# lancedb/lance

Measured on AMD Instinct MI355X. Metric: QPS @ recall@10 (SIFT-1M IVF_PQ nlist=256 M=16) + index-build sec, higher is better.
Workload: dtype f32; 1 GPU; SIFT-1M-like 1Mx128 f32, IVF_PQ nlist=256 M=16 nbits=8, build+search on MI355X; n=1000000, d=128, nlist=256, m=16, k=10, nprobes=10, refine_factor=10, parallelism=single

## Files before the change

### lance_amd/csrc/ctx.cpp

```cpp
#include "common.h"

namespace lh {
static thread_local char g_err[1024] = "";
void set_error(const char *fmt, ...) {
  va_list ap;
  va_start(ap, fmt);
  vsnprintf(g_err, sizeof(g_err), fmt, ap);
  va_end(ap);
}
}

void *lance_hip_ctx::scratch(const char *name, size_t bytes) {
  if (bytes == 0) bytes = 16;
  auto it = slots.find(name);
  if (it != slots.end() && it->second.second >= bytes) return it->second.first;
  if (capturing) {
    lh::set_error("scratch '%s' would have to grow to %zu bytes while a search graph is being captured", name, bytes);
    return nullptr;
  }
  if (it != slots.end()) {
    drop_graphs();
    (void)hipStreamSynchronize(stream);
    (void)hipFree(it->second.first);
    slots.erase(it);
// ... 143 lines not shown
}

int lance_hip_malloc(lance_hip_ctx *ctx, size_t bytes, void **out) {
  lh::CtxLock _ctx_lock(ctx);
  LH_REQUIRE(ctx && out, "malloc: NULL argument");
  LH_CHECK_HIP(hipSetDevice(ctx->device));
  hipError_t e = hipMalloc(out, bytes ? bytes : 16);
  if (e != hipSuccess) {
    lh::set_error("hipMalloc(%zu) failed: %s", bytes, hipGetErrorString(e));
    return LANCE_HIP_ENOMEM;
  }
  return LANCE_HIP_OK;
}
int lance_hip_free(lance_hip_ctx *ctx, void *ptr) {
  lh::CtxLock _ctx_lock(ctx);
  LH_REQUIRE(ctx, "ctx is NULL");
  if (ptr) LH_CHECK_HIP(hipFree(ptr));
  return LANCE_HIP_OK;
}
int lance_hip_memcpy_h2d(lance_hip_ctx *ctx, void *dst, const void *src_host, size_t bytes) {
  lh::CtxLock _ctx_lock(ctx);
  LH_REQUIRE(ctx && (bytes == 0 || (dst && src_host)), "memcpy_h2d: NULL argument");
  if (bytes == 0) return LANCE_HIP_OK;
  LH_CHECK_HIP(hipMemcpyAsync(dst, src_host, bytes, hipMemcpyHostToDevice, ctx->stream));
  LH_CHECK_HIP(hipStreamSynchronize(ctx->stream));
  return LANCE_HIP_OK;
}
int lance_hip_memcpy_d2h(lance_hip_ctx *ctx, void *dst_host, const void *src, size_t bytes) {
  lh::CtxLock _ctx_lock(ctx);
  LH_REQUIRE(ctx && (bytes == 0 || (dst_host && src)), "memcpy_d2h: NULL argument");
  if (bytes == 0) return LANCE_HIP_OK;
  LH_CHECK_HIP(hipMemcpyAsync(dst_host, src, bytes, hipMemcpyDeviceToHost, ctx->stream));
  LH_CHECK_HIP(hipStreamSynchronize(ctx->stream));
  return LANCE_HIP_OK;
}

int lance_hip_timing_enable(lance_hip_ctx *ctx, int on) {
  lh::CtxLock _ctx_lock(ctx);
  LH_REQUIRE(ctx, "ctx is NULL");
  ctx->timing = on != 0;
  return LANCE_HIP_OK;
}

int lance_hip_timing_query(lance_hip_ctx *ctx, const char *kernel, double *ms_total, uint64_t *launches) {
  lh::CtxLock _ctx_lock(ctx);
  LH_REQUIRE(ctx && kernel, "timing_query: NULL argument");
  LH_CHECK_HIP(hipStreamSynchronize(ctx->stream));
  if (strncmp(kernel, "count:", 6) == 0) {
    auto it = ctx->stage_counts.find(kernel + 6);
    if (ms_total) *ms_total = 0.0;
    if (launches) *launches = it == ctx->stage_counts.end() ? 0 : it->second;
    return LANCE_HIP_OK;
  }
  auto &t = ctx->timers[kernel];
  for (auto &ev : t.pending) {
    float ms = 0.f;
    if (hipEventElapsedTime(&ms, ev.first, ev.second) == hipSuccess) {
      t.ms += ms;
      t.launches += 1;
    }
    (void)hipEventDestroy(ev.first);
    (void)hipEventDestroy(ev.second);
  }
  t.pending.clear();
  if (ms_total) *ms_total = t.ms;
  if (launches) *launches = t.launches;
  t.ms = 0.0;
  t.launches = 0;
  return LANCE_HIP_OK;
}

}
```

### lance_amd/csrc/group.hip

```cpp
#include "common.h"
#include "kernels.h"

namespace lh {

constexpr int GROUP_ROWS_PER_BLOCK = 1024;

__global__ __launch_bounds__(64) void group_hist_kernel(const uint32_t *__restrict__ ids, int64_t n, int64_t id_stride,
                                                        int k, int nblocks, uint32_t *__restrict__ blockhist,
                                                        const uint8_t *__restrict__ active) {
  extern __shared__ uint32_t hist[];
  const int b = blockIdx.y;
  if (active && !active[b]) return;
  const int blk = blockIdx.x;
  for (int c = threadIdx.x; c < k; c += 64) hist[c] = 0;
  __syncthreads();
  const uint32_t *idb = ids + (int64_t)b * id_stride;
  const int64_t r0 = (int64_t)blk * GROUP_ROWS_PER_BLOCK;
  for (int ch = 0; ch < GROUP_ROWS_PER_BLOCK / 64; ++ch) {
    const int64_t r = r0 + ch * 64 + threadIdx.x;
    if (r < n) {
      const uint32_t key = idb[r];
      if (key < (uint32_t)k) atomicAdd(&hist[key], 1u);
    }
  }
  __syncthreads();
  uint32_t *out = blockhist + (int64_t)b * k * nblocks;
  for (int c = threadIdx.x; c < k; c += 64) out[(int64_t)c * nblocks + blk] = hist[c];
}

__global__ __launch_bounds__(64) void group_scan_blocks_kernel(uint32_t *__restrict__ blockhist, int k, int nblocks,
                                                               uint32_t *__restrict__ totals,
                                                               const uint8_t *__restrict__ active) {
  const int b = blockIdx.y;
  if (active && !active[b]) return;
  const int c = blockIdx.x;
  uint32_t *h = blockhist + ((int64_t)b * k + c) * nblocks;
  const int lane = threadIdx.x;
  uint32_t carry = 0;
  for (int base = 0; base < nblocks; base += 64) {
    const int i = base + lane;
    const uint32_t v = i < nblocks ? h[i] : 0;
    uint32_t incl = v;
#pragma unroll
    for (int off = 1; off < 64; off <<= 1) {
      const uint32_t t = __shfl_up(incl, off, 64);
      if (lane >= off) incl += t;
    }
    if (i < nblocks) h[i] = carry + incl - v;
    carry += __shfl(incl, 63, 64);
  }
  if (lane == 0) totals[(int64_t)b * k + c] = carry;
}
// ... 99 lines not shown
    if (lane == 63) wsum[wave] = incl;
    __syncthreads();
    uint32_t woff = 0;
    for (int w = 0; w < wave; ++w) woff += wsum[w];
    const uint32_t carry = carry_s;
    if (c < k) st[c] = carry + woff + incl - tot;
    __syncthreads();
    if (threadIdx.x == 255) carry_s = carry + woff + incl;
    __syncthreads();
  }
  if (threadIdx.x == 0) st[k] = carry_s;
}

__global__ __launch_bounds__(64) void group_scatter_kernel(const uint32_t *__restrict__ ids, int64_t n, int64_t id_stride,
                                                           int k, int kbits, int nblocks,
                                                           const uint32_t *__restrict__ blockoffs,
                                                           const uint32_t *__restrict__ starts,
                                                           uint32_t *__restrict__ sorted_rows, int64_t out_stride,
                                                           const uint8_t *__restrict__ active) {
  extern __shared__ uint32_t cursor[];
  const int b = blockIdx.y;
  if (active && !active[b]) return;
  const int blk = blockIdx.x;
  const uint32_t *offs = blockoffs + (int64_t)b * k * nblocks;
  const uint32_t *st = starts + (int64_t)b * (k + 1);
  for (int c = threadIdx.x; c < k; c += 64) cursor[c] = st[c] + offs[(int64_t)c * nblocks + blk];
  __syncthreads();
  const uint32_t *idb = ids + (int64_t)b * id_stride;
  uint32_t *outb = sorted_rows + (int64_t)b * out_stride;
  const int lane = threadIdx.x;
  const uint64_t below = lane == 0 ? 0ull : (~0ull >> (64 - lane));
  const int64_t r0 = (int64_t)blk * GROUP_ROWS_PER_BLOCK;
  for (int ch = 0; ch < GROUP_ROWS_PER_BLOCK / 64; ++ch) {
    const int64_t r = r0 + ch * 64 + lane;
    uint32_t key = LANCE_HIP_NONE;
    if (r < n) key = idb[r];
    const bool valid = key < (uint32_t)k;
    uint64_t mask = __ballot(valid);
    for (int bit = 0; bit < kbits; ++bit) {
      const bool one = (key >> bit) & 1u;
      const uint64_t bal = __ballot(one);
      mask &= one ? bal : ~bal;
    }
    uint32_t base = 0;
    if (valid) base = cursor[key];
    __syncthreads();
    if (valid) {
      const uint32_t rank = (uint32_t)__popcll(mask & below);
      outb[base + rank] = (uint32_t)r;
      if (rank == 0) cursor[key] = base + (uint32_t)__popcll(mask);
    }
    __syncthreads();
  }
}

__global__ __launch_bounds__(256) void group_digit_lo_kernel(const uint32_t *__restrict__ ids, int64_t n, int k, uint32_t *__restrict__ out) {
  const int64_t i = (int64_t)blockIdx.x * 256 + threadIdx.x;
  if (i < n) out[i] = ids[i] < (uint32_t)k ? (ids[i] & 255u) : LANCE_HIP_NONE;
}
__global__ __launch_bounds__(256) void group_digit_hi_kernel(const uint32_t *__restrict__ ids, const uint32_t *__restrict__ p1,
                                                             const uint32_t *__restrict__ nvalid, int64_t n, uint32_t *__restrict__ out) {
  const int64_t j = (int64_t)blockIdx.x * 256 + threadIdx.x;
  if (j < n) out[j] = j < (int64_t)*nvalid ? (ids[p1[j]] >> 8) : LANCE_HIP_NONE;
}
__global__ __launch_bounds__(256) void group_compose_kernel(const uint32_t *__restrict__ p1, const uint32_t *__restrict__ p2,
                                                            const uint32_t *__restrict__ nvalid, int64_t n, uint32_t *__restrict__ out) {
  const int64_t j = (int64_t)blockIdx.x * 256 + threadIdx.x;
  if (j < n && j < (int64_t)*nvalid) out[j] = p1[p2[j]];
}
__global__ __launch_bounds__(256) void group_count_kernel(const uint32_t *__restrict__ ids, int64_t n, int k, uint32_t *__restrict__ counts) {
  const int64_t i = (int64_t)blockIdx.x * 256 + threadIdx.x;
  if (i < n && ids[i] < (uint32_t)k) atomicAdd(&counts[ids[i]], 1u);
}

int stable_group(lance_hip_ctx *ctx, const uint32_t *ids, int64_t n, int64_t id_stride, int k, int batches,
                 uint32_t *starts, uint32_t *sorted_rows, int64_t out_stride, const uint8_t *active);

static int stable_group_wide(lance_hip_ctx *ctx, const uint32_t *ids, int64_t n, int k, uint32_t *starts, uint32_t *sorted_rows) {
  LH_REQUIRE(k <= (1 << 22), "stable_group: k=%d not supported (<= 4194304)", k);
  const int k2 = (k + 255) / 256;
  const size_t nn = (size_t)(n > 0 ? n : 1);
  uint32_t *klo = ctx->scratch_t<uint32_t>("group.klo", nn), *khi = ctx->scratch_t<uint32_t>("group.khi", nn);
  uint32_t *p1 = ctx->scratch_t<uint32_t>("group.p1", nn), *p2 = ctx->scratch_t<uint32_t>("group.p2", nn);
  uint32_t *st1 = ctx->scratch_t<uint32_t>("group.st1", 257), *st2 = ctx->scratch_t<uint32_t>("group.st2", (size_t)k2 + 1);
  uint32_t *counts = ctx->scratch_t<uint32_t>("group.counts", (size_t)k);
  if (!klo || !khi || !p1 || !p2 || !st1 || !st2 || !counts) return LANCE_HIP_ENOMEM;
  const unsigned grid = (unsigned)cdiv(nn, 256);
  hipLaunchKernelGGL(group_digit_lo_kernel, dim3(grid), dim3(256), 0, ctx->stream, ids, n, k, klo);
  LH_TRY(stable_group(ctx, klo, n, n, 256, 1, st1, p1, n, nullptr));
  hipLaunchKernelGGL(group_digit_hi_kernel, dim3(grid), dim3(256), 0, ctx->stream, ids, p1, st1 + 256, n, khi);
  LH_TRY(stable_group(ctx, khi, n, n, k2, 1, st2, p2, n, nullptr));
  hipLaunchKernelGGL(group_compose_kernel, dim3(grid), dim3(256), 0, ctx->stream, p1, p2, st1 + 256, n, sorted_rows);
  LH_CHECK_HIP(lh::memset_async(counts, 0, (size_t)k * 4, ctx->stream));
  hipLaunchKernelGGL(group_count_kernel, dim3(grid), dim3(256), 0, ctx->stream, ids, n, k, counts);
  hipLaunchKernelGGL(group_scan_totals_big_kernel, dim3(1), dim3(256), 0, ctx->stream, counts, k, starts);
  LH_CHECK_HIP(hipGetLastError());
  return LANCE_HIP_OK;
}

int stable_group(lance_hip_ctx *ctx, const uint32_t *ids, int64_t n, int64_t id_stride, int k, int batches,
                 uint32_t *starts, uint32_t *sorted_rows, int64_t out_stride, const uint8_t *active) {
  LH_REQUIRE(k > 0, "stable_group: k=%d not supported", k);
  LH_REQUIRE(n < (1ll << 32), "stable_group: n too large");
  if (batches == 0) return LANCE_HIP_OK;
  if (k > 16384) {
    LH_REQUIRE(batches == 1 && active == nullptr, "stable_group: more than 16384 keys only for a single problem");
    return stable_group_wide(ctx, ids, n, k, starts, sorted_rows);
  }
  const int nblocks = (int)cdiv(n > 0 ? n : 1, GROUP_ROWS_PER_BLOCK);
  uint32_t *blockhist = ctx->scratch_t<uint32_t>("group.blockhist", (size_t)batches * k * nblocks);
  uint32_t *totals = ctx->scratch_t<uint32_t>("group.totals", (size_t)batches * k);
  if (!blockhist || !totals) return LANCE_HIP_ENOMEM;
  int kbits = 0;
  while ((1 << kbits) < k) ++kbits;
  const size_t lds = (size_t)k * sizeof(uint32_t);
  hipLaunchKernelGGL(group_hist_kernel, dim3(nblocks, batches), dim3(64), lds, ctx->stream, ids, n, id_stride, k,
                     nblocks, blockhist, active);
  if (k <= 256 && nblocks <= 256) {
    hipLaunchKernelGGL(group_scan_fused_kernel, dim3(batches), dim3(256), 0, ctx->stream, blockhist, k, nblocks, starts, active);
  } else {
    hipLaunchKernelGGL(group_scan_blocks_kernel, dim3(k, batches), dim3(64), 0, ctx->stream, blockhist, k, nblocks, totals, active);
    hipLaunchKernelGGL(group_scan_totals_kernel, dim3(batches), dim3(256), 0, ctx->stream, totals, k, starts, active);
  }
  hipLaunchKernelGGL(group_scatter_kernel, dim3(nblocks, batches), dim3(64), lds, ctx->stream, ids, n, id_stride, k,
                     kbits, nblocks, blockhist, starts, sorted_rows, out_stride, active);
  LH_CHECK_HIP(hipGetLastError());
  return LANCE_HIP_OK;
}

}
```

### lance_amd/csrc/kernels.h

```cpp
#pragma once
#include <stdint.h>

#include "common.h"

namespace lh {

struct PairwiseArgs {
  const void *x_native = nullptr;
  int x_dtype = 0;
  const float *x = nullptr;
  bool lanes32 = false;
  int64_t n = 0;
  int64_t ldx = 0;
  int x_batch_off = 0;
  const float *cent = nullptr;
  int k = 0;
  int64_t cent_batch_stride = 0;
  const float *bias = nullptr;
  int64_t bias_batch_stride = 0;
  uint32_t *ids = nullptr;
  float *dists = nullptr;
  int64_t out_batch_stride = 0;
  uint8_t *codes = nullptr;
  int codes_ld = 0;
// ... 26 lines not shown
int launch_pq_mfma_encode(lance_hip_ctx *ctx, int dtype, const void *x, int64_t n, int d, const float *cent, const uint32_t *part_ids,
                          int residual, const float *codebook, int m, uint8_t *codes);

struct FlatPool {
  const float *x;
  const void *x_native = nullptr;
  int x_dtype = 0;
  const uint64_t *row_ids;
  int64_t r0, r1;
  const float *q;
  int nq, k, cap;
  uint32_t *tkey;
  uint64_t *trid;
  uint32_t *cnt;
  uint32_t *pkeys;
  uint64_t *prids;
  uint32_t *overflow;
  const float *row_sy = nullptr;
  const float *q_norm = nullptr;
};

int launch_wide_filter(lance_hip_ctx *ctx, const FlatPool &fp, int d, int metric);
int build_allow_bits(lance_hip_ctx *ctx, const uint64_t *row_ids, uint64_t n, const uint8_t *allow_by_rowid, uint64_t n_allow, const uint32_t **bits_out);
bool flat_mfma_supported(int metric, int d, int nq, const void *x, const float *q);
int flat_mfma_prepare(lance_hip_ctx *ctx, const float *q, int nq, int d, const uint16_t **qhi, const uint16_t **qlo, const float **qn);
int launch_flat_filter_mfma(lance_hip_ctx *ctx, const FlatPool &e, int d, int metric, const uint16_t *qhi, const uint16_t *qlo, const float *qn);
bool flat_mfma_wide_supported(int metric, int d, int nq, int64_t n, const float *x, const float *q);
int flat_mfma_wide_prepare_rows(lance_hip_ctx *ctx, const float *x, int64_t n, int d, const uint16_t **xb, const float **xn2);
int flat_mfma_wide_prepare_queries(lance_hip_ctx *ctx, const float *q, int nq, int d, const uint16_t **qb, const float **qn2);
int launch_flat_filter_mfma_wide(lance_hip_ctx *ctx, const FlatPool &e, int d, int metric, const uint16_t *xb, const float *xn2, const uint16_t *qb,
                                 const float *qn2);

int launch_assign(lance_hip_ctx *ctx, const PairwiseArgs &p, int d, int metric, int batches);
bool assign_reads_native(PairwiseArgs p, int d, int batches);
bool encode_fused_supported(int dtype, int d, int m, int nbits, const void *x, const float *cent, const float *codebook);
int launch_encode_fused(lance_hip_ctx *ctx, int dtype, const void *x, int64_t n, int d, const float *cent, const uint32_t *part_ids,
                        int residual, const float *codebook, int m, uint8_t *codes);
bool xform_fused_supported(int dtype, int metric, int d, int m, int nbits, int64_t n, int nlist, const void *x, const float *cent,
                           const float *codebook, uint8_t *codes, bool lanes32);
int launch_xform_fused(lance_hip_ctx *ctx, int dtype, int metric, const void *x, int64_t n, int d, const float *cent, int nlist,
                       const float *codebook, int m, uint32_t *part_ids, float *dists, uint8_t *codes, bool round_f16);
bool xform_tail_supported(int d, int m, int nbits, int64_t n, const float *x, const float *cent, const float *codebook);
int launch_xform_tail(lance_hip_ctx *ctx, const float *x, int64_t n, int d, const float *cent, const uint32_t *part_ids, int residual, bool round_f16,
                      const float *codebook, int m, uint8_t *codes);
bool xform_pqtrain_supported(const PairwiseArgs &p, int sd, int batches);
int launch_xform_pqtrain(lance_hip_ctx *ctx, const PairwiseArgs &p, int sd, int batches, uint32_t *fb_cnt, uint32_t *fb_items);
bool xform_assign_supported(const PairwiseArgs &p, int d, int metric, int batches);
int launch_xform_assign(lance_hip_ctx *ctx, const PairwiseArgs &p, int d, int metric);
int launch_xform_sweep_groups(lance_hip_ctx *ctx, int metric, const float *q, uint32_t nq, int d, const float *cent, uint32_t nlist, uint32_t *maxbits,
                              float *gkey, int ng, float *e2, const uint16_t *cpl_ready = nullptr, const uint32_t *maxbits_ready = nullptr);
size_t xform_coarse_planes_elems(uint32_t nlist, int d);
int xform_coarse_planes(lance_hip_ctx *ctx, int metric, const float *cent, uint32_t nlist, int d, uint16_t *cpl, uint32_t *maxbits );
bool coarse_groups_shape(int d, uint32_t nlist);
bool mfma_assign_supported(const PairwiseArgs &p, int d, int batches);
int launch_assign_mfma(lance_hip_ctx *ctx, const PairwiseArgs &p, int d, int metric);
int launch_dist_matrix(lance_hip_ctx *ctx, const PairwiseArgs &p, int d, int metric, int batches);

int stable_group(lance_hip_ctx *ctx, const uint32_t *ids, int64_t n, int64_t id_stride, int k, int batches,
                 uint32_t *starts, uint32_t *sorted_rows, int64_t out_stride, const uint8_t *active);

int kmeans_train_batched(lance_hip_ctx *ctx, int metric, const float *x, int64_t n, int64_t ldx, int x_batch_off, int d,
                         int k, int B, uint32_t max_iters, double tol, float balance_factor_scaled, bool have_init,
                         const uint64_t *seeds, float *cent, double *loss_out, uint32_t *iters_out, bool f16_arith = false);

int kmeans_train_hierarchical(lance_hip_ctx *ctx, int metric, const float *x, int64_t n, int d, int target_k, uint32_t max_iters,
                              double tol, float bf_scaled, int hierarchical_k, uint64_t seed, float *cent_out, uint32_t *n_out,
                              bool f16_arith = false);
int check_dtype(int dtype, const char *what);
int model_dtype(int dtype);
int as_f32(lance_hip_ctx *ctx, int dtype, const void *p, size_t count, const char *slot, const float **out);
int widen_into(lance_hip_ctx *ctx, int dtype, const void *p, size_t count, float *dst);
int from_f32(lance_hip_ctx *ctx, int dtype, const float *src, void *dst, size_t count);
int launch_residual(lance_hip_ctx *ctx, const float *x, int64_t n, int d, const float *cent, const uint32_t *part_ids, float *out, bool f16);


bool pm_supported(const lance_hip_index *ix, uint32_t keff, int has_range, uint32_t nq, uint32_t nprobes);
int ivfpq_scan_merge_pm(lance_hip_ctx *ctx, const lance_hip_index *ix, const float *qs, uint32_t nq, const uint32_t *probes,
                        uint32_t nprobes, uint32_t keff, uint32_t k, bool do_refine, uint64_t *ids, float *dists,
                        uint64_t *cand_rid, uint32_t *cand_cnt, uint32_t *flags, const uint32_t *allow);
int find_partitions_f32(lance_hip_ctx *ctx, int metric, const float *qf, uint32_t nq, uint32_t d, const float *cf, uint32_t nlist,
                        uint32_t nprobes, uint32_t *part_ids, float *dists, bool lanes32);
bool flat_small_supported(int metric, int dtype, uint32_t d, uint32_t nq, uint32_t k, uint64_t n);
int flat_topk_small(lance_hip_ctx *ctx, int metric, int dtype, const void *x, const uint64_t *row_ids, uint64_t n, uint32_t d, const float *q,
                    uint32_t nq, uint32_t k, uint64_t *ids, float *dists, bool *done);
bool coarse_mfma_supported(int metric, int d, uint32_t nq, uint32_t nlist, uint32_t nprobes, bool lanes32, const float *q, const float *cent);
int find_partitions_mfma(lance_hip_ctx *ctx, int metric, const float *q, uint32_t nq, int d, const float *cent, uint32_t nlist, uint32_t nprobes,
                         float *matrix, uint32_t *part_ids, float *dists, const uint16_t *cpl_ready = nullptr, const uint32_t *maxbits_ready = nullptr);
int launch_normalize(lance_hip_ctx *ctx, const float *x, int64_t n, int d, float *out, bool f16);
int launch_normalize_planes(lance_hip_ctx *ctx, const float *x, int64_t n, int d, float *out, bool f16, uint16_t *plane16, int dp, float *n2);

int qscan_index_constants(lance_hip_ctx *ctx, lance_hip_index *ix);
constexpr int QSCAN_SEG_CAP = 256;
struct SelectOut;
bool qscan_supported(const lance_hip_index *ix, uint32_t nq, uint32_t nprobes);
bool qscan_tiled_shape(int m, int sd);
int qscan_classb_to_rescan(lance_hip_ctx *ctx, const uint32_t *tbound, uint32_t nq, uint32_t nprobes, uint32_t *seg_cnt, uint32_t *qovf);
int qscan_nearest_keys(lance_hip_ctx *ctx, const uint32_t *probes, uint32_t nq, uint32_t nprobes, uint32_t *keys, uint32_t nb = 1);
int qscan_item_tables(lance_hip_ctx *ctx, const uint32_t *pair_starts, int nlist, int G, uint32_t *item_start, int4 *desc, uint32_t max_items);
int qscan_group(lance_hip_ctx *ctx, const uint32_t *probes, uint32_t nq, uint32_t nprobes, int nlist, const uint32_t *tglobal,
                uint32_t *keys, uint32_t *tbound, uint32_t *pair_starts, uint32_t *pair_idx, uint32_t *item_start4, int4 *desc4,
                uint32_t max_items4, int G = 4, int dot = 0);
int qbound_launch(lance_hip_ctx *ctx, const lance_hip_index *ix, const float *qs, uint32_t nq, uint32_t keff, const uint32_t *pair_starts0,
                  const uint32_t *pair_idx0, uint32_t *item_start, int4 *desc, uint32_t max_items, uint32_t *tglobal, const uint32_t *allow);
int qscan_launch(lance_hip_ctx *ctx, const lance_hip_index *ix, const float *qs, uint32_t nq, uint32_t nprobes, const uint32_t *pair_idx,
                 const uint32_t *item_start4, const int4 *desc4, uint32_t max_items4, const uint32_t *tbound, uint32_t *seg_cnt,
                 uint32_t *seg_pos, uint32_t *qovf, const uint32_t *allow, const uint32_t *probes = nullptr);
bool qscan_pt_enabled(const lance_hip_index *ix);
int qscan_pt_mode(const lance_hip_index *ix);
int qbound_pt_launch(lance_hip_ctx *ctx, const lance_hip_index *ix, const float *qs, uint32_t nq, uint32_t nprobes, uint32_t keff,
                     const uint32_t *probes, const uint32_t *pair_starts0, const uint32_t *pair_idx0, uint32_t *item_start, int4 *desc,
                     uint32_t max_items, uint32_t *tglobal, const uint32_t *allow);
int qmerge_launch(lance_hip_ctx *ctx, const lance_hip_index *ix, const float *qs, uint32_t nq, const uint32_t *probes, uint32_t nprobes,
// ... 20 lines not shown
```

### lance_amd/csrc/mfma_assign.hip

```cpp
#include <algorithm>
#include <cstdlib>
#include <cstring>

#include <hip/hip_fp16.h>

#include "common.h"
#include "exact.cuh"
#include "kernels.h"
#include "ma_common.cuh"

#pragma clang fp contract(off)

namespace lh {

__global__ __launch_bounds__(64) void ma_prep_kernel(const float *__restrict__ cent, int k, int d, int dp, const float *__restrict__ bias,
                                                     uint16_t *__restrict__ chi, uint16_t *__restrict__ clo, float *__restrict__ cn,
                                                     uint32_t *__restrict__ maxbits ,
                                                     const uint8_t *__restrict__ active) {
  if (active && !active[0]) return;
  const int c = blockIdx.x;
  float s = 0.0f;
  for (int e = threadIdx.x; e < dp; e += 64) {
    const float v = e < d ? cent[(int64_t)c * d + e] : 0.0f;
    const uint32_t hb = bf16_rne_bits(v);
// ... 798 lines not shown
    case 5: ok = ma_launch_ks<5>(ctx, a, metric, dtype, p.lanes32); break;
    case 6: ok = ma_launch_ks<6>(ctx, a, metric, dtype, p.lanes32); break;
    case 7: ok = ma_launch_ks<7>(ctx, a, metric, dtype, p.lanes32); break;
    case 8: ok = ma_launch_ks<8>(ctx, a, metric, dtype, p.lanes32); break;
    default: return LANCE_HIP_EINVAL;
  }
  LH_REQUIRE(ok, "assign: element type %d with metric %d is not on the MFMA path", dtype, metric);
  LH_CHECK_HIP(hipGetLastError());
  return LANCE_HIP_OK;
}

constexpr int CS_CAP = 128;
constexpr int CS_CAP_G = 512;

template <int METRIC>
__device__ __forceinline__ float cs_group_distance(const float *wrow, const float *__restrict__ y, int d, int lane) {
  const int i = lane & 15, full = d / 16 * 16;
  float s = 0.0f, acc = 0.0f;
  if (full != d) {
    float r = 0.0f;
    for (int e = full; e < d; ++e) {
      if constexpr (METRIC == METRIC_DOT) r = r + wrow[e] * y[e];
      else { const float diff = wrow[e] - y[e]; r = r + diff * diff; }
    }
    s = r;
  }
  int ch = 0;
  for (; ch + 128 <= full; ch += 128) {
    float yv[8];
#pragma unroll
    for (int u = 0; u < 8; ++u) yv[u] = y[ch + 16 * u + i];
#pragma unroll
    for (int u = 0; u < 8; ++u) {
      const float xv = wrow[ch + 16 * u + i];
      if constexpr (METRIC == METRIC_DOT) acc = acc + xv * yv[u];
      else { const float diff = xv - yv[u]; acc = acc + diff * diff; }
    }
  }
  for (; ch < full; ch += 16) {
    const float xv = wrow[ch + i], yv = y[ch + i];
    if constexpr (METRIC == METRIC_DOT) acc = acc + xv * yv;
    else { const float diff = xv - yv; acc = acc + diff * diff; }
  }
  float run = 0.0f + acc;
#pragma unroll
  for (int t = 1; t < 16; ++t) {
    const float prev = __builtin_bit_cast(float, __builtin_amdgcn_update_dpp(0, __builtin_bit_cast(int, run), 0x111, 0xF, 0xF, false));
    run = prev + acc;
  }
  const float tot = __shfl(run, (lane & 48) + 15, 64);
  return finish_metric<METRIC>(s + tot);
}

template <int METRIC, bool GROUPS = false>
__global__ __launch_bounds__(256) void coarse_select_kernel(float *__restrict__ sur, const float *__restrict__ e2, const float *__restrict__ q,
                                                            const float *__restrict__ cent, int nq, int nlist, int d, int nprobes,
                                                            uint32_t *__restrict__ part_ids, float *__restrict__ dists,
                                                            uint32_t *__restrict__ n_exact_rows, const float *__restrict__ gkey = nullptr,
                                                            const float *__restrict__ gsec = nullptr, int ng = 0) {
  extern __shared__ __attribute__((aligned(16))) char smem[];
  const int lane = threadIdx.x & 63, wave = threadIdx.x >> 6, grp = lane >> 4;
  const int qi = blockIdx.x * 4 + wave;
  if (qi >= nq) return;
  const int dpad = (d + 3) & ~3;
  constexpr int CAP = GROUPS ? CS_CAP_G : CS_CAP;
  float *wrow = reinterpret_cast<float *>(smem) + (size_t)wave * dpad;
  unsigned long long *ck = reinterpret_cast<unsigned long long *>(smem + (size_t)4 * dpad * 4) + (size_t)wave * CAP;
  uint32_t *cl = reinterpret_cast<uint32_t *>(smem + (size_t)4 * dpad * 4 + (size_t)4 * CAP * 8) + (size_t)wave * CAP;
  const float *qv = q + (int64_t)qi * d;
  for (int e = lane; e < d; e += 64) wrow[e] = qv[e];
  float *row = sur + (int64_t)qi * nlist;
  const float E2 = GROUPS ? e2[qi] * 1.0625f : e2[qi];
  const float *gk = GROUPS ? gkey + (int64_t)qi * 2 * ng : nullptr;
  float m0 = INFINITY, m1 = INFINITY, m2 = INFINITY, m3 = INFINITY;
  bool bad = !(E2 < INFINITY) || !(E2 > 7.888609052210118e-31f);
  auto ins4 = [&](float v) {
    if (v < m3) {
      if (v < m2) {
        m3 = m2;
        if (v < m1) {
          m2 = m1;
          if (v < m0) { m1 = m0; m0 = v; } else m1 = v;
        } else m2 = v;
      } else m3 = v;
    }
  };
  if constexpr (GROUPS) {
    for (int i = lane * 4; i < 2 * ng; i += 256) {
      const f4 v = *reinterpret_cast<const f4 *>(gk + i);
      bad |= (v.x != v.x) | (v.y != v.y);
      ins4(v.x); ins4(v.y);
    }
  } else {
  for (int i = lane; i < nlist; i += 64) {
    const float v = row[i];
    bad |= v != v;
    ins4(v);
  }
  }
  bad = __any(bad);
  float sv4[4] = {m0, m1, m2, m3};
#pragma unroll
  for (int k2 = 2; k2 <= 256; k2 <<= 1) {
#pragma unroll
    for (int dd = k2 >> 1; dd > 0; dd >>= 1) {
      if (dd >= 64) {
        const int jd = dd >> 6;
#pragma unroll
        for (int jr = 0; jr < 4; ++jr) {
          if ((jr & jd) == 0) {
            const bool up = ((jr * 64) & k2) == 0;
            const float lo = fminf(sv4[jr], sv4[jr | jd]), hi = fmaxf(sv4[jr], sv4[jr | jd]);
            sv4[jr] = up ? lo : hi; sv4[jr | jd] = up ? hi : lo;
          }
        }
      } else {
#pragma unroll
        for (int jr = 0; jr < 4; ++jr) {
          const int e = jr * 64 + lane;
          const float o = __shfl_xor(sv4[jr], dd, 64);
          const bool up = (e & k2) == 0, lower = (lane & dd) == 0;
          sv4[jr] = (lower == up) ? fminf(sv4[jr], o) : fmaxf(sv4[jr], o);
        }
      }
    }
  }
// ... 67 lines not shown
    for (int r = 0; r < nprobes; ++r) {
      unsigned long long best = ~0ull;
      for (int i = lane; i < nlist; i += 64) {
        const unsigned long long kk = ((unsigned long long)order_key(row[i]) << 32) | (uint32_t)i;
        if ((!have_last || kk > last) && kk < best) best = kk;
      }
#pragma unroll
      for (int o = 32; o > 0; o >>= 1) { const unsigned long long ob = __shfl_xor(best, o, 64); best = ob < best ? ob : best; }
      if (lane == 0) {
        part_ids[(int64_t)qi * nprobes + r] = (uint32_t)best;
        if (dists) dists[(int64_t)qi * nprobes + r] = key_to_float((uint32_t)(best >> 32));
      }
      last = best; have_last = true;
    }
    return;
  }
  for (uint32_t c0 = 0; c0 < cnt; c0 += 4) {
    const uint32_t ci = c0 + (uint32_t)grp;
    const uint32_t c = ci < cnt ? cl[ci] : cl[0];
    const float v = cs_group_distance<METRIC>(wrow, cent + (int64_t)c * d, d, lane);
    if (ci < cnt && (lane & 15) == 0) ck[ci] = ((unsigned long long)order_key(v) << 32) | c;
  }
  __builtin_amdgcn_wave_barrier();
  unsigned long long v2[2];
  v2[0] = (uint32_t)lane < cnt ? ck[lane] : ~0ull;
  for (uint32_t base = 64;; base += 64) {
    v2[1] = base + (uint32_t)lane < cnt ? ck[base + (uint32_t)lane] : ~0ull;
#pragma unroll
    for (int k2 = 2; k2 <= 128; k2 <<= 1) {
#pragma unroll
      for (int dd = k2 >> 1; dd > 0; dd >>= 1) {
        if (dd >= 64) {
          const unsigned long long a = v2[0], b = v2[1];
          if (a > b) { v2[0] = b; v2[1] = a; }
        } else {
#pragma unroll
          for (int jr = 0; jr < 2; ++jr) {
            const int e = jr * 64 + lane;
            const unsigned long long o = __shfl_xor(v2[jr], dd, 64);
            const bool up = (e & k2) == 0, lower = (lane & dd) == 0;
            v2[jr] = (lower == up) ? (v2[jr] < o ? v2[jr] : o) : (v2[jr] > o ? v2[jr] : o);
          }
        }
      }
    }
    if (base + 64 >= cnt) break;
  }
  if (lane < nprobes) {
    part_ids[(int64_t)qi * nprobes + lane] = (uint32_t)v2[0];
    if (dists) dists[(int64_t)qi * nprobes + lane] = key_to_float((uint32_t)(v2[0] >> 32));
  }
}

bool coarse_mfma_supported(int metric, int d, uint32_t nq, uint32_t nlist, uint32_t nprobes, bool lanes32, const float *q, const float *cent) {
  static const char *env = getenv("LANCE_HIP_MFMA_COARSE");
  static const bool off = env && env[0] == '0', force = env && env[0] == '1';
  if (off || lanes32 || (metric != METRIC_L2 && metric != METRIC_DOT)) return false;
  if (nprobes == 0 || nprobes > 64 || nprobes > nlist) return false;
  if ((reinterpret_cast<uintptr_t>(q) | reinterpret_cast<uintptr_t>(cent)) & 15) return false;
  if (d <= 128) { if (d % 16 != 0 || d < 16 || nlist < 32) return false; }
  else if (d > 4096 || nlist < 64 || d % 4 != 0) return false;
  if (force) return true;
  if (d > 128) return (uint64_t)nq * nlist >= (1ull << 23);
  return (uint64_t)nq * nlist * (uint64_t)d >= (1ull << 27);
}

template <int KS>
static void coarse_launch_narrow(lance_hip_ctx *ctx, const MaArgs &a, int metric, dim3 grid) {
  constexpr int D = KS * 16;
  const size_t lds_x = (size_t)MA_ROWS * (D + 4) * 4;
  const size_t lds_c = (size_t)2 * 2 * MA_CT * (D + 8) * 2 + (size_t)2 * 2 * MA_CT * 4;
  const size_t lds = std::max(lds_x, lds_c);
  if (a.gkey) {
    if (metric == METRIC_DOT) hipLaunchKernelGGL((ma_top3_kernel<KS, METRIC_DOT, float, 2>), grid, dim3(256), lds, ctx->stream, a);
    else hipLaunchKernelGGL((ma_top3_kernel<KS, METRIC_L2, float, 2>), grid, dim3(256), lds, ctx->stream, a);
    return;
  }
  if (metric == METRIC_DOT) hipLaunchKernelGGL((ma_top3_kernel<KS, METRIC_DOT, float, 1>), grid, dim3(256), lds, ctx->stream, a);
  else hipLaunchKernelGGL((ma_top3_kernel<KS, METRIC_L2, float, 1>), grid, dim3(256), lds, ctx->stream, a);
}

static int coarse_groups_from() {
  static const int v = getenv("LANCE_HIP_COARSE_GROUPS") ? atoi(getenv("LANCE_HIP_COARSE_GROUPS")) : 1024;
  return v;
}
bool coarse_groups_shape(int d, uint32_t nlist) {
  static const bool ma = getenv("LANCE_HIP_COARSE_GROUPS_MA") != nullptr;
  return !ma && d <= 128 && d % 16 == 0 && coarse_groups_from() > 0 && nlist >= (uint32_t)std::max(coarse_groups_from(), 256);
}

int find_partitions_mfma(lance_hip_ctx *ctx, int metric, const float *q, uint32_t nq, int d, const float *cent, uint32_t nlist, uint32_t nprobes,
                         float *matrix, uint32_t *part_ids, float *dists, const uint16_t *cpl_ready, const uint32_t *maxbits_ready) {
  const bool wide = d > 128;
  const int dp = wide ? (d + MW_KC - 1) / MW_KC * MW_KC : d;
  const size_t kd = (size_t)nlist * dp;
  uint16_t *chi = ctx->scratch_t<uint16_t>("cq.chi", kd), *clo = ctx->scratch_t<uint16_t>("cq.clo", kd);
  float *cn = ctx->scratch_t<float>("cq.cn", (size_t)nlist);
  uint32_t *maxbits = ctx->scratch_t<uint32_t>("cq.maxbits", 4);
  float *e2 = ctx->scratch_t<float>("cq.e2", (size_t)nq);
  if (!chi || !clo || !cn || !maxbits || !e2) return LANCE_HIP_ENOMEM;
  const int groups_from = coarse_groups_from();
  const bool groups = !wide && groups_from > 0 && nlist >= (uint32_t)std::max(groups_from, 256);
  const int ng = groups ? (int)cdiv(nlist, MA_CT) * 4 : 0;
  float *gkey = nullptr, *gsec = nullptr;
  if (groups) {
    gkey = ctx->scratch_t<float>("cq.gkey", (size_t)nq * 2 * ng);
    gsec = gkey;
    if (!gkey) return LANCE_HIP_ENOMEM;
  }
  LH_CHECK_HIP(lh::memset_async(maxbits, 0, 16, ctx->stream));
  static const bool groups_ma = getenv("LANCE_HIP_COARSE_GROUPS_MA") != nullptr;
  if (groups && !groups_ma) {
    ScopedTimer t(ctx, "dist_matrix");
    LH_TRY(launch_xform_sweep_groups(ctx, metric, q, nq, d, cent, nlist, maxbits, gkey, ng, e2, cpl_ready, maxbits_ready));
  } else {
    ScopedTimer t(ctx, "dist_matrix");
    hipLaunchKernelGGL(ma_prep_kernel, dim3(nlist), dim3(64), 0, ctx->stream, cent, (int)nlist, d, dp, nullptr, chi, clo, cn, maxbits, nullptr);
    MaArgs a;
    a.x = q; a.n = nq; a.ldx = d; a.d = d; a.k = (int)nlist;
    a.chi = chi; a.clo = clo; a.cn = cn; a.bias = nullptr; a.maxbits = maxbits; a.cent = cent;
    a.sur = matrix; a.e2 = e2; a.active = nullptr;
    a.gkey = gkey; a.gsec = gsec; a.ng = ng;
    const unsigned rblocks = (unsigned)cdiv(nq, wide ? MW_ROWS : MA_ROWS);
    const int ntiles = (int)cdiv(nlist, wide ? MW_CT : MA_CT);
    int slices = (int)std::min<uint64_t>((uint64_t)ntiles, std::max<uint64_t>(1, ((uint64_t)2 * ctx->num_cus) / rblocks));
    a.tiles_per_block = (int)cdiv((uint64_t)ntiles, (uint64_t)slices);
    slices = (int)cdiv((uint64_t)ntiles, (uint64_t)a.tiles_per_block);
    const dim3 grid(rblocks, (unsigned)slices);
    if (wide) {
      uint16_t *xhi = ctx->scratch_t<uint16_t>("cq.xhi", (size_t)nq * dp), *xlo = ctx->scratch_t<uint16_t>("cq.xlo", (size_t)nq * dp);
      float *xn2 = ctx->scratch_t<float>("cq.xn2", (size_t)nq);
      if (!xhi || !xlo || !xn2) return LANCE_HIP_ENOMEM;
      a.xhi = xhi; a.xlo = xlo; a.xn2 = xn2; a.dp = dp;
      hipLaunchKernelGGL((ma_split_rows_kernel<float>), dim3((unsigned)cdiv(nq, 4)), dim3(256), 0, ctx->stream, q, (int64_t)nq, (int64_t)d, d, dp, xhi, xlo,
                         xn2, nullptr);
      if (metric == METRIC_DOT) hipLaunchKernelGGL((ma_top3_wide_kernel<METRIC_DOT, true>), grid, dim3(256), 0, ctx->stream, a);
      else hipLaunchKernelGGL((ma_top3_wide_kernel<METRIC_L2, true>), grid, dim3(256), 0, ctx->stream, a);
    } else {
      switch (d / 16) {
        case 1: coarse_launch_narrow<1>(ctx, a, metric, grid); break;
        case 2: coarse_launch_narrow<2>(ctx, a, metric, grid); break;
        case 3: coarse_launch_narrow<3>(ctx, a, metric, grid); break;
        case 4: coarse_launch_narrow<4>(ctx, a, metric, grid); break;
        case 5: coarse_launch_narrow<5>(ctx, a, metric, grid); break;
        case 6: coarse_launch_narrow<6>(ctx, a, metric, grid); break;
        case 7: coarse_launch_narrow<7>(ctx, a, metric, grid); break;
        case 8: coarse_launch_narrow<8>(ctx, a, metric, grid); break;
        default: return LANCE_HIP_EINVAL;
      }
    }
  }
  {
    ScopedTimer t(ctx, "select_probes");
    const int dpad = (d + 3) & ~3;
    const int cap = groups ? CS_CAP_G : CS_CAP;
    const size_t lds = (size_t)4 * dpad * 4 + (size_t)4 * cap * 8 + (size_t)4 * cap * 4;
    if (groups) {
      ctx->count_stage("coarse_groups");
      if (metric == METRIC_DOT)
        hipLaunchKernelGGL((coarse_select_kernel<METRIC_DOT, true>), dim3((unsigned)cdiv(nq, 4)), dim3(256), lds, ctx->stream, matrix, e2, q, cent, (int)nq,
                           (int)nlist, d, (int)nprobes, part_ids, dists, maxbits + 2, gkey, gsec, ng);
      else
        hipLaunchKernelGGL((coarse_select_kernel<METRIC_L2, true>), dim3((unsigned)cdiv(nq, 4)), dim3(256), lds, ctx->stream, matrix, e2, q, cent, (int)nq,
                           (int)nlist, d, (int)nprobes, part_ids, dists, maxbits + 2, gkey, gsec, ng);
    } else if (metric == METRIC_DOT)
      hipLaunchKernelGGL((coarse_select_kernel<METRIC_DOT>), dim3((unsigned)cdiv(nq, 4)), dim3(256), lds, ctx->stream, matrix, e2, q, cent, (int)nq, (int)nlist,
                         d, (int)nprobes, part_ids, dists, maxbits + 2);
    else
      hipLaunchKernelGGL((coarse_select_kernel<METRIC_L2>), dim3((unsigned)cdiv(nq, 4)), dim3(256), lds, ctx->stream, matrix, e2, q, cent, (int)nq, (int)nlist,
                         d, (int)nprobes, part_ids, dists, maxbits + 2);
  }
  static const bool stats = getenv("LANCE_HIP_COARSE_STATS") != nullptr;
  if (stats && !ctx->capturing) {
    uint32_t h[4];
    LH_CHECK_HIP(hipMemcpyAsync(h, maxbits, 16, hipMemcpyDeviceToHost, ctx->stream));
    LH_CHECK_HIP(hipStreamSynchronize(ctx->stream));
    fprintf(stderr, "[coarse] nq=%u nlist=%u nprobes=%u groups=%d: %u queries took the exact path\n", nq, nlist, nprobes, groups ? 1 : 0, h[2]);
  }
  LH_CHECK_HIP(hipGetLastError());
  return LANCE_HIP_OK;
}

}
```

### lance_amd/csrc/search.hip

```cpp
#include <algorithm>
#include <cstdlib>
#include <string>
#include <vector>

#include "common.h"
#include "exact.cuh"
#include "index.h"
#include "kernels.h"
#include "search_common.cuh"

#pragma clang fp contract(off)

namespace lh {

#ifndef LH_SCAN_CAP
#define LH_SCAN_CAP 1024
#endif
#ifndef LH_SCAN_ROUND
#define LH_SCAN_ROUND 512
#endif
#ifndef LH_LUT_BATCH
#define LH_LUT_BATCH 4
#endif
constexpr int SCAN_CAP = LH_SCAN_CAP;
// ... 851 lines not shown
            }
          }
      }
    }
    float oth[8];
#pragma unroll
    for (int e = 0; e < 8; ++e) oth[e] = __shfl_xor(acc[e], 1, 64);
    if (h == 0 && i < P) {
      float tot = 0.0f;
#pragma unroll
      for (int e = 0; e < 8; ++e) tot = tot + acc[e];
#pragma unroll
      for (int e = 0; e < 8; ++e) tot = tot + oth[e];
      tot = 0.0f + tot;
      key[i] = ok ? order_key(finish_metric<METRIC>(tot)) : 0xFFFFFFFFu;
      rid[i] = r; pos[i] = 0;
    }
  }
  __syncthreads();
  refine_write_cand_exact(cand_exact, key, keff, c, qi);
  refine_emit_topk(key, rid, pos, P, c, k, qi, out_ids, out_dists);
}

__global__ __launch_bounds__(256) void raw_to_u8_kernel(const f4 *__restrict__ x, int64_t n16, uint4 *__restrict__ out, uint32_t *__restrict__ bad) {
  bool ok = true;
  for (int64_t i = (int64_t)blockIdx.x * 256 + threadIdx.x; i < n16; i += (int64_t)gridDim.x * 256) {
    uint32_t w[4];
#pragma unroll
    for (int p = 0; p < 4; ++p) {
      const f4 v = x[i * 4 + p];
      uint32_t pk = 0;
#pragma unroll
      for (int e = 0; e < 4; ++e) {
        const uint32_t b = (v[e] >= 0.0f && v[e] < 256.0f) ? (uint32_t)v[e] : 0u;
        ok = ok && (float)b == v[e];
        pk |= b << (8 * e);
      }
      w[p] = pk;
    }
    out[i] = make_uint4(w[0], w[1], w[2], w[3]);
  }
  if (__any(!ok) && (threadIdx.x & 63) == 0) atomicOr(bad, 1u);
}

static bool raw_compact_enabled() {
  static const bool off = getenv("LANCE_HIP_NO_RAW_COMPACT") != nullptr;
  return !off;
}
int coarse_planes_prepare(lance_hip_ctx *ctx, const lance_hip_index *ix_c, int scan_metric) {
  lance_hip_index *ix = const_cast<lance_hip_index *>(ix_c);
  std::lock_guard<std::mutex> lk(ix->lazy_mu);
  if (ix->cq || ctx->capturing) return LANCE_HIP_OK;
  auto *cq = new lance_hip_index::CqConst();
  bool ok = hipMalloc(reinterpret_cast<void **>(&cq->cpl), xform_coarse_planes_elems(ix->nlist, (int)ix->d) * 2) == hipSuccess;
  ok = ok && hipMalloc(reinterpret_cast<void **>(&cq->maxbits), 16) == hipSuccess;
  auto drop = [&]() { if (cq->cpl) (void)hipFree(cq->cpl); if (cq->maxbits) (void)hipFree(cq->maxbits); delete cq; };
  if (!ok) { (void)hipGetLastError(); drop(); return LANCE_HIP_OK; }
  if (lh::memset_async(cq->maxbits, 0, 16, ctx->stream) != hipSuccess ||
      xform_coarse_planes(ctx, scan_metric, ix->centroids, ix->nlist, (int)ix->d, cq->cpl, cq->maxbits) != LANCE_HIP_OK ||
      hipStreamSynchronize(ctx->stream) != hipSuccess) {
    drop();
    set_error("find_partitions: building the centroid planes of the index failed");
    return LANCE_HIP_ERUNTIME;
  }
  ix->cq = cq;
  return LANCE_HIP_OK;
}

const uint8_t *raw_compact_prepare(lance_hip_ctx *ctx, const lance_hip_index *ix_c) {
  lance_hip_index *ix = const_cast<lance_hip_index *>(ix_c);
  if (!raw_compact_enabled() || ix->dtype != LANCE_HIP_F32 || !ix->raw || ix->n_raw == 0 || (ix->d & 15) != 0 ||
      (ix->metric != LANCE_HIP_L2 && ix->metric != LANCE_HIP_DOT) || (reinterpret_cast<uintptr_t>(ix->raw) & 15) != 0)
    return nullptr;
  std::lock_guard<std::mutex> lk(ix->lazy_mu);
  if (ix->raw_compact_state != 0) return ix->raw_compact_state > 0 ? ix->raw_u8 : nullptr;
  if (ctx->capturing) return nullptr;
  const uint64_t bytes = ix->n_raw * (uint64_t)ix->d;
  uint8_t *buf = nullptr;
  uint32_t *bad = ctx->scratch_t<uint32_t>("raw.compact_flag", 1);
  if (!bad || hipMalloc(reinterpret_cast<void **>(&buf), bytes) != hipSuccess) {
    (void)hipGetLastError();
    ix->raw_compact_state = -1;
    return nullptr;
  }
  uint32_t bad_h = 1;
  bool ran = lh::memset_async(bad, 0, 4, ctx->stream) == hipSuccess;
  if (ran) {
    const int64_t n16 = (int64_t)(bytes / 16);
    hipLaunchKernelGGL(raw_to_u8_kernel, dim3((unsigned)std::min<uint64_t>(cdiv((uint64_t)n16, 256), 1u << 20)), dim3(256), 0, ctx->stream,
                       static_cast<const f4 *>(ix->raw), n16, reinterpret_cast<uint4 *>(buf), bad);
    ran = hipGetLastError() == hipSuccess && hipMemcpyAsync(&bad_h, bad, 4, hipMemcpyDeviceToHost, ctx->stream) == hipSuccess &&
          hipStreamSynchronize(ctx->stream) == hipSuccess;
  }
  if (!ran || bad_h != 0) {
    (void)hipFree(buf);
    ix->raw_compact_state = -1;
    return nullptr;
  }
  ix->raw_u8 = buf;
  ix->raw_compact_state = 1;
  return buf;
}


struct ExactArgs {
  ScanArgs s;
  const uint64_t *row_ids;
  int k, refine;
  uint64_t *out_ids;
  float *out_dists;
  uint64_t *cand_rid;
  uint32_t *cand_cnt;
// ... 321 lines not shown
    }
    for (int i = 0; i < 4 && hipGetLastError() != hipSuccess; ++i) {}
  }
  set_error("");
  int prc = plain();
  if (prc == LANCE_HIP_ERUNTIME) {
    (void)hipStreamSynchronize(ctx->stream);
    for (int i = 0; i < 4 && hipGetLastError() != hipSuccess; ++i) {}
    set_error("");
    prc = plain();
  }
  return prc;
}

static int ivfpq_search_enqueue_impl(lance_hip_ctx *ctx, const lance_hip_index *ix, const float *q, uint32_t nq, uint32_t k,
                                     uint32_t nprobes, uint32_t refine_factor, int has_range, float lower, float upper,
                                     uint64_t *ids, float *dists, uint32_t **flags_out, const uint32_t *allow) {
  LH_REQUIRE(k > 0, "search: k must be > 0");
  if (nprobes > ix->nlist) nprobes = ix->nlist;
  LH_REQUIRE(ix->nlist <= 8192 || nprobes <= 2048, "search: nprobes=%u > 2048 with more than 8192 partitions is not supported", nprobes);
  LH_REQUIRE(nprobes > 0, "search: nprobes must be > 0");
  const uint32_t rf = refine_factor == 0 ? 1 : refine_factor;
  const uint64_t keff64 = (uint64_t)k * rf;
  LH_REQUIRE(keff64 <= 8192, "search: k * refine_factor = %llu > 8192 is not supported", (unsigned long long)keff64);
  const uint32_t keff = (uint32_t)keff64;
  const bool fast = keff <= (uint32_t)SCAN_MAX_KEFF;
  const bool do_refine = refine_factor >= 1;
  LH_REQUIRE(!do_refine || ix->raw != nullptr, "search: refine_factor needs raw vectors (lance_hip_index_set_raw)");
  const int d = (int)ix->d, m = (int)ix->m, sd = d / m, nlist = (int)ix->nlist;
  const int scan_metric = ix->metric == LANCE_HIP_COSINE ? LANCE_HIP_L2 : ix->metric;

  uint32_t *flags = ctx->scratch_t<uint32_t>("search.flags", (size_t)nq + 1);
  if (!flags) return LANCE_HIP_ENOMEM;
  LH_CHECK_HIP(lh::memset_async(flags, 0, ((size_t)nq + 1) * 4, ctx->stream));
  uint32_t *n_fallback = flags + nq;
  ctx->last_replay_counter = n_fallback;
  if (flags_out) *flags_out = flags;
  if (nq == 0) return LANCE_HIP_OK;

  const float *qs = q;
  if (ix->metric == LANCE_HIP_COSINE) {
    float *qn = ctx->scratch_t<float>("search.qnorm", (size_t)nq * d);
    if (!qn) return LANCE_HIP_ENOMEM;
    LH_TRY(launch_normalize(ctx, q, (int64_t)nq, d, qn, ix->dtype == LANCE_HIP_F16));
    qs = qn;
  }
  float *matrix = ctx->scratch_t<float>("search.matrix", (size_t)nq * nlist);
  uint32_t *probes = ctx->scratch_t<uint32_t>("search.probes", (size_t)nq * nprobes);
  if (!matrix || !probes) return LANCE_HIP_ENOMEM;
  const bool coarse_l32 = ix->dtype == LANCE_HIP_F16 && scan_metric == LANCE_HIP_DOT && d > 16;
  if (coarse_mfma_supported(scan_metric, d, nq, (uint32_t)nlist, nprobes, coarse_l32, qs, ix->centroids)) {
    const uint16_t *cpl = nullptr;
    const uint32_t *cmb = nullptr;
    if (coarse_groups_shape(d, (uint32_t)nlist)) {
      LH_TRY(coarse_planes_prepare(ctx, ix, scan_metric));
      if (ix->cq) { cpl = ix->cq->cpl; cmb = ix->cq->maxbits; }
    }
    LH_TRY(find_partitions_mfma(ctx, scan_metric, qs, nq, d, ix->centroids, (uint32_t)nlist, nprobes, matrix, probes, nullptr, cpl, cmb));
  } else {
    PairwiseArgs pa;
    pa.x = qs; pa.n = nq; pa.ldx = d; pa.cent = ix->centroids; pa.k = nlist; pa.matrix = matrix;
    pa.lanes32 = coarse_l32;
    LH_TRY(launch_dist_matrix(ctx, pa, d, scan_metric, 1));
    ScopedTimer t(ctx, "select_probes");
    launch_select_probes(ctx, matrix, nlist, (int)nprobes, (int)nq, probes, nullptr);
  }
  uint64_t *cand_rid = nullptr;
  uint32_t *cand_cnt = nullptr;
  if (do_refine) {
    cand_rid = ctx->scratch_t<uint64_t>("search.cand_rid", (size_t)nq * keff);
    cand_cnt = ctx->scratch_t<uint32_t>("search.cand_cnt", nq);
    if (!cand_rid || !cand_cnt) return LANCE_HIP_ENOMEM;
  }
  static const bool no_pm = getenv("LANCE_HIP_NO_PM") != nullptr;
  const uint64_t pm_min_pairs = qscan_tiled_shape(m, sd) ? 2048 : 4096;
  const bool use_pm = fast && !no_pm && pm_supported(ix, keff, has_range, nq, nprobes) && (uint64_t)nq * nprobes >= pm_min_pairs;
  int nsplit = 1;
  if (nq < (uint32_t)(2 * ctx->num_cus)) {
    nsplit = (int)std::min<uint64_t>({8ull, (uint64_t)nprobes, cdiv(2ull * ctx->num_cus, nq)});
    if (nsplit < 1) nsplit = 1;
  }
  const size_t nblk = (size_t)nq * nsplit;
  uint32_t *ckeys = nullptr, *cpos = nullptr, *ccnt = nullptr;
  if (!use_pm) {
    ckeys = ctx->scratch_t<uint32_t>("search.ckeys", nblk * SCAN_LCAP);
    cpos = ctx->scratch_t<uint32_t>("search.cpos", nblk * SCAN_LCAP);
    ccnt = ctx->scratch_t<uint32_t>("search.ccnt", nblk);
    if (!ckeys || !cpos || !ccnt) return LANCE_HIP_ENOMEM;
  }
  ScanArgs a;
  {
    a.q = qs; a.probes = probes; a.centroids = ix->centroids; a.codebook = ix->codebook;
    a.part_offsets = ix->part_offsets; a.codes = ix->codes;
    a.d = d; a.m = m; a.sd = sd; a.nprobes = (int)nprobes; a.nsplit = nsplit; a.keff = (int)keff;
    a.nbits = (int)ix->nbits;
    a.residual = scan_metric == LANCE_HIP_L2 ? 1 : 0;
    a.round_f16 = ix->dtype == LANCE_HIP_F16 ? 1 : 0;
    a.lanes32 = (ix->dtype == LANCE_HIP_F16 && scan_metric == LANCE_HIP_DOT && sd > 16) ? 1 : 0;
    a.has_range = has_range;
    a.allow = allow;
    a.lo_key = 0; a.hi_key = 0xFFFFFFFFu;
    if (has_range) {
      uint32_t lb, ub;
      memcpy(&lb, &lower, 4); memcpy(&ub, &upper, 4);
      a.lo_key = (lb & 0x80000000u) ? ~lb : (lb | 0x80000000u);
      a.hi_key = (ub & 0x80000000u) ? ~ub : (ub | 0x80000000u);
    }
// ... 53 lines not shown

int find_partitions_f32(lance_hip_ctx *ctx, int metric, const float *qf, uint32_t nq, uint32_t d, const float *cf, uint32_t nlist,
                        uint32_t nprobes, uint32_t *part_ids, float *dists, bool lanes32) {
  if (nprobes > nlist) nprobes = nlist;
  LH_REQUIRE(nlist <= 8192 || nprobes <= 2048, "find_partitions: nprobes=%u > 2048 with more than 8192 partitions is not supported", nprobes);
  if (nq == 0 || nprobes == 0) return LANCE_HIP_OK;
  float *matrix = ctx->scratch_t<float>("search.matrix", (size_t)nq * nlist);
  if (!matrix) return LANCE_HIP_ENOMEM;
  const int km = metric == LANCE_HIP_COSINE ? LANCE_HIP_L2 : metric;
  if (coarse_mfma_supported(km, (int)d, nq, nlist, nprobes, lanes32, qf, cf)) {
    LH_TRY(find_partitions_mfma(ctx, km, qf, nq, (int)d, cf, nlist, nprobes, matrix, part_ids, dists));
  } else {
    PairwiseArgs pa;
    pa.x = qf; pa.n = nq; pa.ldx = d;
    pa.cent = cf; pa.k = (int)nlist; pa.matrix = matrix;
    pa.lanes32 = lanes32;
    LH_TRY(launch_dist_matrix(ctx, pa, (int)d, km, 1));
    launch_select_probes(ctx, matrix, (int)nlist, (int)nprobes, (int)nq, part_ids, dists);
  }
  LH_CHECK_HIP(hipGetLastError());
  LH_CHECK_HIP(hipStreamSynchronize(ctx->stream));
  return LANCE_HIP_OK;
}

static int check_flags(lance_hip_ctx *ctx, const uint32_t *flags, uint32_t nq) {
  std::vector<uint32_t> fh(nq);
  LH_CHECK_HIP(hipMemcpyAsync(fh.data(), flags, (size_t)nq * 4, hipMemcpyDeviceToHost, ctx->stream));
  LH_CHECK_HIP(hipStreamSynchronize(ctx->stream));
  uint32_t n_over = 0, n_amb = 0, n_bad = 0;
  for (uint32_t i = 0; i < nq; ++i) { n_over += (fh[i] & FLAG_OVERFLOW) ? 1 : 0; n_amb += (fh[i] & FLAG_AMBIGUOUS) ? 1 : 0; n_bad += (fh[i] & FLAG_BADROW) ? 1 : 0; }
  if (n_bad) {
    set_error("search: refine met row ids beyond the %s raw vectors given to lance_hip_index_set_raw (%u queries): the raw array must be "
              "indexed by the stored row ids", "attached", n_bad);
    return LANCE_HIP_EINVAL;
  }
  if (n_over || n_amb) {
    set_error("search: internal error, %u overflow / %u ambiguous queries were not resolved by the exact kernel", n_over, n_amb);
    return LANCE_HIP_ERUNTIME;
  }
  return LANCE_HIP_OK;
}

}

using namespace lh;

extern "C" {

int lance_hip_index_prewarm(lance_hip_ctx *ctx, lance_hip_index *idx) {
  lh::CtxLock _ctx_lock(ctx);
  LH_REQUIRE(ctx && idx, "index_prewarm: NULL argument");
  LH_CHECK_HIP(hipSetDevice(ctx->device));
  if (idx->m > 0 && idx->nbits == 8) LH_TRY(mscan_prewarm(ctx, idx));
  if (coarse_groups_shape((int)idx->d, idx->nlist) && (reinterpret_cast<uintptr_t>(idx->centroids) & 15) == 0)
    LH_TRY(coarse_planes_prepare(ctx, idx, idx->metric == LANCE_HIP_COSINE ? LANCE_HIP_L2 : idx->metric));
  (void)raw_compact_prepare(ctx, idx);
  LH_CHECK_HIP(hipStreamSynchronize(ctx->stream));
  return LANCE_HIP_OK;
}

int lance_hip_find_partitions(lance_hip_ctx *ctx, int dtype, int metric, const void *q, uint32_t nq, uint32_t d,
                              const void *centroids, uint32_t nlist, uint32_t nprobes, uint32_t *part_ids, float *dists) {
  lh::CtxLock _ctx_lock(ctx);
  LH_REQUIRE(ctx && q && centroids && part_ids, "find_partitions: NULL argument");
  LH_TRY(check_dtype(dtype, "find_partitions"));
  LH_REQUIRE(nlist > 0 && nlist <= 65536, "find_partitions: nlist=%u not supported in this version (1..65536)", nlist);
  LH_CHECK_HIP(hipSetDevice(ctx->device));
  const float *qf, *cf;
  LH_TRY(as_f32(ctx, dtype, q, (size_t)nq * d, "f16.q", &qf));
  LH_TRY(as_f32(ctx, model_dtype(dtype), centroids, (size_t)nlist * d, "f16.cent", &cf));
  return find_partitions_f32(ctx, metric, qf, nq, d, cf, nlist, nprobes, part_ids, dists, dtype == LANCE_HIP_F16 && metric == LANCE_HIP_DOT && d > 16);
}

int lance_hip_ivfpq_search_async(lance_hip_ctx *ctx, const lance_hip_index *idx, const void *q, uint32_t nq, uint32_t k,
                                 uint32_t nprobes, uint32_t refine_factor, uint64_t *ids, float *dists) {
  lh::CtxLock _ctx_lock(ctx);
  LH_REQUIRE(ctx && idx && (nq == 0 || (q && ids && dists)), "search: NULL argument");
  LH_REQUIRE(ctx->device == idx->device, "search: context and index live on different devices");
  LH_CHECK_HIP(hipSetDevice(ctx->device));
  const float *qf;
  LH_TRY(as_f32(ctx, idx->dtype, q, (size_t)nq * idx->d, "f16.q", &qf));
  return ivfpq_search_enqueue(ctx, idx, qf, nq, k, nprobes, refine_factor, 0, 0.f, 0.f, ids, dists, nullptr, nullptr);
}

int lance_hip_ivfpq_search(lance_hip_ctx *ctx, const lance_hip_index *idx, const void *q, uint32_t nq, uint32_t k,
                           uint32_t nprobes, uint32_t refine_factor, uint64_t *ids, float *dists) {
  lh::CtxLock _ctx_lock(ctx);
  LH_REQUIRE(ctx && idx && (nq == 0 || (q && ids && dists)), "search: NULL argument");
  LH_REQUIRE(ctx->device == idx->device, "search: context and index live on different devices");
  LH_CHECK_HIP(hipSetDevice(ctx->device));
  uint32_t *flags = nullptr;
  const float *qf;
  LH_TRY(as_f32(ctx, idx->dtype, q, (size_t)nq * idx->d, "f16.q", &qf));
  LH_TRY(ivfpq_search_enqueue(ctx, idx, qf, nq, k, nprobes, refine_factor, 0, 0.f, 0.f, ids, dists, &flags, nullptr));
  return check_flags(ctx, flags, nq);
}

int lance_hip_ivfpq_search_candidates(lance_hip_ctx *ctx, const lance_hip_index *idx, const void *q, uint32_t nq, uint32_t keff, uint32_t nprobes,
                                      uint64_t *ids, float *pq_dists, float *exact_dists) {
  lh::CtxLock _ctx_lock(ctx);
  LH_REQUIRE(ctx && idx && (nq == 0 || (q && ids && pq_dists)), "search_candidates: NULL argument");
  LH_REQUIRE(ctx->device == idx->device, "search_candidates: context and index live on different devices");
  LH_REQUIRE(idx->m != 0, "search_candidates: not an IVF_PQ index");
  LH_REQUIRE(!exact_dists || idx->raw != nullptr, "search_candidates: exact distances need raw vectors (lance_hip_index_set_raw)");
  LH_CHECK_HIP(hipSetDevice(ctx->device));
  if (nq == 0) return LANCE_HIP_OK;
  uint32_t *flags = nullptr;
// ... 136 lines not shown
```

### lance_amd/csrc/search_common.cuh

```cuda
#pragma once
#include <hip/hip_runtime.h>
#include <stdint.h>

#include "exact.cuh"

namespace lh {

constexpr uint32_t FLAG_OVERFLOW = 1u, FLAG_AMBIGUOUS = 2u, FLAG_BADROW = 4u;
constexpr int SCAN_LCAP = 256;
constexpr int SCAN_MAX_KEFF = 128;

__device__ __forceinline__ bool row_allowed(const uint32_t *__restrict__ allow, uint32_t pos) {
  return allow == nullptr || ((allow[pos >> 5] >> (pos & 31u)) & 1u) != 0u;
}

static inline int next_pow2(int v) { int p = 1; while (p < v) p <<= 1; return p; }

__device__ __forceinline__ uint32_t find_partition_dev(const uint32_t *__restrict__ offs, int nlist, uint32_t slot) {
  int lo = 0, hi = nlist;
  while (hi - lo > 1) {
    const int mid = (lo + hi) >> 1;
    if (offs[mid] <= slot) lo = mid; else hi = mid;
  }
  return (uint32_t)lo;
}

template <int BS = 256>
__device__ __forceinline__ void bitonic_sort_kr(uint32_t *key, uint64_t *rid, uint32_t *pos, int P) {
  for (int k2 = 2; k2 <= P; k2 <<= 1) {
    for (int j = k2 >> 1; j > 0; j >>= 1) {
      for (int i = threadIdx.x; i < P / 2; i += BS) {
        const int ix = 2 * j * (i / j) + (i % j);
        const int px = ix + j;
        const bool up = (ix & k2) == 0;
        const uint32_t kx = key[ix], ky = key[px];
        const uint64_t rx = rid[ix], ry = rid[px];
        const bool gt = kx > ky || (kx == ky && rx > ry);
        if (gt == up) {
          key[ix] = ky; key[px] = kx; rid[ix] = ry; rid[px] = rx;
          const uint32_t t = pos[ix]; pos[ix] = pos[px]; pos[px] = t;
        }
      }
      __syncthreads();
    }
  }
}

struct SelectOut {
  int keff, k, refine;
  uint64_t *out_ids;
  float *out_dists;
  uint64_t *cand_rid;
  uint32_t *cand_cnt;
  uint32_t *flags;
  const uint32_t *part_offsets;
  int nlist;
};

template <int BS = 256>
__device__ __forceinline__ void select_and_emit(const SelectOut &o, int q, uint32_t *key, uint64_t *rid, uint32_t *pos, int total,
                                                int *s_amb) {
  const int got = min(total, o.keff);
  if (total > o.keff && key[o.keff] == key[o.keff - 1]) {
    const uint32_t tf = key[o.keff - 1];
    int lo = o.keff, hi = total;
    while (lo < hi) { const int mid = (lo + hi) >> 1; if (key[mid] <= tf) lo = mid + 1; else hi = mid; }
    const int L = lo;
    for (int i = threadIdx.x; i < L; i += BS) {
      const uint32_t pi = find_partition_dev(o.part_offsets, o.nlist, pos[i]);
      const uint32_t a = o.part_offsets[pi], b = o.part_offsets[pi + 1];
      int same = 0;
      for (int j = 0; j < L; ++j) same += (pos[j] >= a && pos[j] < b) ? 1 : 0;
      if (same > o.keff) *s_amb = 1;
    }
    __syncthreads();
    if (threadIdx.x == 0 && *s_amb) atomicOr(&o.flags[q], FLAG_AMBIGUOUS);
  }
// ... 46 lines not shown
```

### lance_amd/csrc/search_ms.hip

```cpp
#include <algorithm>
#include <cmath>
#include <cstdio>
#include <cstdlib>
#include <cstring>
#include <vector>

#include "common.h"
#include "exact.cuh"
#include "index.h"
#include "kernels.h"
#include "search_common.cuh"
#include "q_common.cuh"

namespace lh {

typedef _Float16 ms_h8 __attribute__((ext_vector_type(8)));
typedef _Float16 ms_h4 __attribute__((ext_vector_type(4)));
typedef float ms_f16v __attribute__((ext_vector_type(16)));

constexpr float MS_SE = 30000.0f;
constexpr float MS_SLACK_CAP = 1500.0f;
constexpr int MS_CUT_SHIFT = 6;
typedef __attribute__((address_space(1))) const void *ms_gptr;
typedef __attribute__((address_space(3))) void *ms_lptr;
// ... 212 lines not shown
    uint32_t v = 0;
    if (i < nlist) {
      const uint32_t qp = pair_starts[i + 1] - pair_starts[i], np = part_offsets[i + 1] - part_offsets[i];
      const MsSplit sp = ms_split(qp, np, rs_rows, rs2_rows);
      v = sp.npb * sp.nrs;
      for (uint32_t pb = 0; pb < sp.npb; pb += max(1u, sp.npb - 1u)) {
        const uint32_t pairs = min(sp.blk, qp - pb * sp.blk), npb_same = (pb + 1 == sp.npb) ? 1u : sp.npb - 1u;
        if (sp.nrs > 0) atomicAdd(&hist[ms_work_class(ms_row_count(0u, np, rs_rows, rs2_rows), pairs, cls_rows)], npb_same);
        if (sp.nrs > 2) atomicAdd(&hist[ms_work_class(rs2_rows, pairs, cls_rows)], npb_same * (sp.nrs - 2u));
        if (sp.nrs > 1) atomicAdd(&hist[ms_work_class(ms_row_count(sp.nrs - 1u, np, rs_rows, rs2_rows), pairs, cls_rows)], npb_same);
        if (sp.npb == 1) break;
      }
    }
    uint32_t incl = v;
#pragma unroll
    for (int off = 1; off < 64; off <<= 1) {
      const uint32_t t = __shfl_up(incl, off, 64);
      if (lane >= off) incl += t;
    }
    if (lane == 63) wsum[wave] = incl;
    __syncthreads();
    uint32_t woff = 0;
    for (int w = 0; w < wave; ++w) woff += wsum[w];
    const uint32_t carry = carry_s;
    if (i < nlist) slice_start[i] = carry + woff + incl - v;
    __syncthreads();
    if (threadIdx.x == 255) carry_s = carry + woff + incl;
    __syncthreads();
  }
  if (threadIdx.x == 0) {
    slice_start[nlist] = carry_s;
    uint32_t run = 0;
    for (int c = 0; c < 32; ++c) { cls_cursor[c] = run; run += hist[c]; }
  }
}

__global__ __launch_bounds__(256) void ms_slice_desc_kernel(const uint32_t *__restrict__ slice_start, const uint32_t *__restrict__ pair_starts,
                                                            const uint32_t *__restrict__ part_offsets, int nlist, uint32_t rs_rows, uint32_t rs2_rows, uint32_t cls_rows,
                                                            MsSlice *__restrict__ slices, uint32_t *__restrict__ cls_cursor, uint32_t *__restrict__ order) {
  const int part = blockIdx.x * 4 + (threadIdx.x >> 6), lane = threadIdx.x & 63;
  if (part >= nlist) return;
  const uint32_t s0 = slice_start[part], s1 = slice_start[part + 1];
  if (s1 == s0) return;
  const uint32_t off = part_offsets[part], np = part_offsets[part + 1] - off;
  const uint32_t gs = pair_starts[part], qp = pair_starts[part + 1] - gs;
  const MsSplit sp = ms_split(qp, np, rs_rows, rs2_rows);
  for (uint32_t t = (uint32_t)lane; t < s1 - s0; t += 64u) {
    const uint32_t pb = t / sp.nrs, rs = t - pb * sp.nrs;
    MsSlice u;
    u.off = off; u.np = np; u.row_begin = ms_row_begin(rs, rs_rows, rs2_rows); u.row_count = ms_row_count(rs, np, rs_rows, rs2_rows);
    u.gs = gs + pb * sp.blk; u.qp = min(sp.blk, qp - pb * sp.blk); u.pad0 = u.pad1 = 0u;
    slices[s0 + t] = u;
    order[atomicAdd(&cls_cursor[ms_work_class(u.row_count, u.qp, cls_rows)], 1u)] = s0 + t;
  }
}

struct MscanArgs {
  const uint32_t *order;
  const MsSlice *slices;
  const uint32_t *slice_start;
  uint32_t *slice_ctr;
  const uint8_t *codes;
  const _Float16 *cbh;
  const float *row_cn2;
  const _Float16 *rh;
  const f4 *prm;
  const f2 *prm2;
  uint32_t nan_slot;
  int nlist, nprobes;
  uint32_t *seg_cnt, *seg_pos;
  uint2 *seg_pv = nullptr;
  uint32_t *ovf;
  const uint32_t *allow;
#ifdef LH_TIMING_EXPERIMENTS
  int dbg = 0;
#endif
  unsigned long long *prof_slices = nullptr;
  unsigned long long *prof = nullptr;
};

#ifdef LH_TIMING_EXPERIMENTS
#define MS_DBG(p) ((p).dbg)
#else
#define MS_DBG(p) 0
#endif

constexpr int MS_QH = 64;
template <int SD, int KS, bool PROF = false>
__global__ __launch_bounds__(1024, 4) void ivfpq_mscan_kernel(MscanArgs p) {
  constexpr int D = KS * 16;
  constexpr int M = D / SD;
  constexpr int RB = D * 2;
  constexpr int CPR = RB / 16;
  constexpr int RPK = 256 / RB;
  constexpr int SPI = 16384 / RB;
  __shared__ __attribute__((aligned(16))) char sB[MS3_PB * RB];
  __shared__ __attribute__((aligned(16))) float sLim[MS3_PB];
  __shared__ __attribute__((aligned(16))) uint32_t sPair[MS3_PB];
  __shared__ __attribute__((aligned(8))) uint2 sQ[16][2][MS_QH + 1];
  __shared__ uint32_t s_slice, s_chunk;
  const int lane = threadIdx.x & 63, wave = __builtin_amdgcn_readfirstlane((int)(threadIdx.x >> 6));
  const int j = lane & 31, g = lane >> 5;
  const uint32_t nslices = p.slice_start[p.nlist];

  uint2 *const qw = &sQ[wave][0][0];
  uint32_t cur = 0;
// ... 541 lines not shown
    mc->sum_rs += rs; mc->max_rs = std::max(mc->max_rs, rs);
  }
  if (hipGetLastError() != hipSuccess || hipStreamSynchronize(ctx->stream) != hipSuccess) {
    drop();
    set_error("matrix-core scan: building the index constants failed");
    return LANCE_HIP_ERUNTIME;
  }
  if (dot) {
    float rm; memcpy(&rm, &rowmax_bits, 4);
    mc->cmax = (float)(std::sqrt((double)rm) / (double)mc->sigma * 1.0001);
    if (!(mc->cmax > 0.0f) || !std::isfinite(mc->cmax)) mc->cmax = mc->cmax_full;
  }
  mc->usable = true;
  ix->ms = mc;
  return LANCE_HIP_OK;
}

int mscan_launch(lance_hip_ctx *ctx, const lance_hip_index *ix_c, const float *qs, uint32_t nq, uint32_t nprobes, const uint32_t *probes,
                 const uint32_t *pair_starts, const uint32_t *pair_idx, const uint32_t *tbound, uint32_t *seg_cnt, uint32_t *seg_pos,
                 uint32_t *qovf, const uint32_t *allow, uint32_t **qslack_out, float **seg_val_out, float **seg_scale_out) {
  lance_hip_index *ix = const_cast<lance_hip_index *>(ix_c);
  int sd = 0, ks = 0;
  if (!ms_shape(ix, &sd, &ks)) return LH_NOT_TAKEN;
  LH_TRY(mscan_prepare(ctx, ix));
  if (!ix->ms->usable) return LH_NOT_TAKEN;
  const int d = (int)ix->d, nlist = (int)ix->nlist;
  const size_t npairs = (size_t)nq * nprobes;
  const uint64_t cap = (uint64_t)ix->ms->sum_rs + (uint64_t)ix->ms->max_rs * cdiv(npairs, MS3_PB) + 8;
  _Float16 *rh = reinterpret_cast<_Float16 *>(ctx->scratch("ms.rh", (npairs + 32) * (size_t)d * 2));
  f4 *prm = reinterpret_cast<f4 *>(ctx->scratch("ms.prm", (npairs + 32) * 16));
  f2 *prm2 = reinterpret_cast<f2 *>(ctx->scratch("ms.prm2", npairs * 8));
  uint32_t *qslack = ctx->scratch_t<uint32_t>("ms.qslack", nq);
  uint32_t *slice_start = ctx->scratch_t<uint32_t>("ms.slice_start", (size_t)nlist + 2 + 32);
  MsSlice *slices = reinterpret_cast<MsSlice *>(ctx->scratch("ms.slices", cap * sizeof(MsSlice)));
  uint32_t *order = ctx->scratch_t<uint32_t>("ms.order", cap);
  float *seg_val = ctx->scratch_t<float>("ms.seg_val", npairs * Q_CAP * 2);
  uint32_t *ovf = ctx->scratch_t<uint32_t>("q.ovf", npairs + 1);
  if (!rh || !prm || !prm2 || !qslack || !slice_start || !slices || !order || !seg_val || !ovf) return LANCE_HIP_ENOMEM;
  uint32_t *slice_ctr = slice_start + nlist + 1, *cls_cursor = slice_ctr + 1;
  const uint32_t nan_slot = (uint32_t)npairs + 1u;
  {
    ScopedTimer t(ctx, "q_residual");
    LH_CHECK_HIP(lh::memset_multi(ctx->stream, {{seg_cnt, 0, npairs * 4}, {qovf, 0, (size_t)nq * 4}, {qslack, 0, (size_t)nq * 4}, {ovf, 0, 4}}));
    MsPrepArgs pa;
    pa.q = qs; pa.centroids = ix->centroids; pa.pair_idx = pair_idx; pa.pair_starts = pair_starts; pa.probes = probes; pa.tbound = tbound;
    pa.d = d; pa.nprobes = (int)nprobes; pa.nlist = nlist; pa.round_f16 = ix->dtype == LANCE_HIP_F16 ? 1 : 0;
    pa.sigma = ix->ms->sigma; pa.rh = rh; pa.prm = prm; pa.qslack = qslack; pa.seg_cnt = seg_cnt; pa.qovf = qovf; pa.ovf = ovf;
    pa.nan_slot = nan_slot; pa.prm2 = prm2;
    pa.dot = ix->metric == LANCE_HIP_DOT ? 1 : 0; pa.cmax = ix->ms->cmax; pa.cmax_full = ix->ms->cmax_full; pa.cmaxp = ix->ms->cmaxp; pa.mu = ix->cb_mean; pa.m = (int)ix->m;
    hipLaunchKernelGGL(ms_prep_kernel, dim3((unsigned)cdiv(npairs, 4 * MS_PPW)), dim3(256), 0, ctx->stream, pa);
    const uint32_t rs_rows = (uint32_t)ms_rows_per_slice(), rs2_rows = (uint32_t)ms_rows_per_slice2();
    static const bool no_order = getenv("LANCE_HIP_MS_NOORDER") != nullptr;
    const uint32_t cls_rows = no_order ? 0x40000000u : rs_rows;
    hipLaunchKernelGGL(ms_slice_table_kernel, dim3(1), dim3(256), 0, ctx->stream, pair_starts, ix->part_offsets, nlist, rs_rows, rs2_rows, cls_rows, slice_start,
                       slice_ctr, cls_cursor);
    hipLaunchKernelGGL(ms_slice_desc_kernel, dim3((unsigned)cdiv((uint64_t)nlist, 4)), dim3(256), 0, ctx->stream, slice_start, pair_starts, ix->part_offsets,
                       nlist, rs_rows, rs2_rows, cls_rows, slices, cls_cursor, order);
  }
  ScopedTimer t(ctx, "ivfpq_scan_c1");
  ScopedTimer tm(ctx, "ivfpq_mscan");
  MscanArgs a;
  a.order = order; a.slices = slices; a.slice_start = slice_start; a.slice_ctr = slice_ctr; a.codes = ix->codes;
  a.cbh = reinterpret_cast<const _Float16 *>(ix->ms->cbh); a.row_cn2 = ix->ms->row_cn2; a.rh = rh; a.prm = prm; a.prm2 = prm2;
  a.nan_slot = nan_slot; a.nlist = nlist; a.nprobes = (int)nprobes;
  a.seg_cnt = seg_cnt; a.seg_pos = seg_pos; a.seg_pv = reinterpret_cast<uint2 *>(seg_val); a.ovf = ovf; a.allow = allow;
#ifdef LH_TIMING_EXPERIMENTS
  static const int dbg = [] {
    const int v = getenv("LANCE_HIP_MS_DBG") ? atoi(getenv("LANCE_HIP_MS_DBG")) : 0;
    if (v) fprintf(stderr, "lance_hip: LANCE_HIP_MS_DBG=%d -- timing experiment, search RESULTS ARE WRONG\n", v);
    return v;
  }();
  a.dbg = dbg;
#endif
  static const int grid_env = getenv("LANCE_HIP_MS_GRID") ? atoi(getenv("LANCE_HIP_MS_GRID")) : 0;
  const unsigned grid = (unsigned)std::min<uint64_t>((uint64_t)(grid_env > 0 ? std::min(grid_env, ctx->num_cus) : ctx->num_cus), cap);
  static const bool prof = getenv("LANCE_HIP_MS_PROF") != nullptr;
  if (prof && sd == 8 && ks == 8 && !ctx->capturing) {
    a.prof = ctx->scratch_t<unsigned long long>("ms.prof", 8);
    if (!a.prof) return LANCE_HIP_ENOMEM;
    LH_CHECK_HIP(lh::memset_async(a.prof, 0, 64, ctx->stream));
    a.prof_slices = ctx->scratch_t<unsigned long long>("ms.prof_slices", cap);
    if (!a.prof_slices) return LANCE_HIP_ENOMEM;
    LH_CHECK_HIP(lh::memset_async(a.prof_slices, 0, cap * 8, ctx->stream));
    hipLaunchKernelGGL((ivfpq_mscan_kernel<8, 8, true>), dim3(grid), dim3(1024), 0, ctx->stream, a);
    unsigned long long h[8];
    LH_CHECK_HIP(hipMemcpyAsync(h, a.prof, 64, hipMemcpyDeviceToHost, ctx->stream));
    LH_CHECK_HIP(hipStreamSynchronize(ctx->stream));
    {
      std::vector<unsigned long long> st(cap);
      std::vector<MsSlice> sl(cap);
      std::vector<uint32_t> ord(cap), ss((size_t)nlist + 1);
      (void)hipMemcpy(st.data(), a.prof_slices, cap * 8, hipMemcpyDeviceToHost);
      (void)hipMemcpy(sl.data(), slices, cap * sizeof(MsSlice), hipMemcpyDeviceToHost);
      (void)hipMemcpy(ord.data(), order, cap * 4, hipMemcpyDeviceToHost);
      (void)hipMemcpy(ss.data(), slice_start, ((size_t)nlist + 1) * 4, hipMemcpyDeviceToHost);
      const uint32_t ns = ss[nlist];
      std::vector<uint32_t> idx(ns);
      for (uint32_t i = 0; i < ns; ++i) idx[i] = i;
      std::sort(idx.begin(), idx.end(), [&](uint32_t x, uint32_t y) { return st[x] > st[y]; });
      double tot = 0, totw = 0;
      for (uint32_t i = 0; i < ns; ++i) { tot += (double)st[i]; totw += (double)sl[ord[i]].row_count * sl[ord[i]].qp; }
      fprintf(stderr, "[ms prof] %u slices, mean %.0f ticks, mean ticks per 1000 cells %.2f; slowest (taken#, ticks, rows, pairs, ticks per 1000 cells):", ns, tot / ns, tot / totw * 1e3);
      for (uint32_t t = 0; t < std::min<uint32_t>(ns, 12); ++t) {
        const uint32_t i = idx[t];
        fprintf(stderr, " (%u, %llu, %u, %u, %.2f)", i, st[i], sl[ord[i]].row_count, sl[ord[i]].qp, (double)st[i] / ((double)sl[ord[i]].row_count * sl[ord[i]].qp) * 1e3);
      }
      fprintf(stderr, " | last taken:");
      for (uint32_t i = ns > 12 ? ns - 12 : 0; i < ns; ++i)
        fprintf(stderr, " (%u, %llu, %u, %u)", i, st[i], sl[ord[i]].row_count, sl[ord[i]].qp);
      fprintf(stderr, "\n");
// ... 55 lines not shown
```

### lance_amd/csrc/search_pm.hip

```cpp
#include <algorithm>
#include <cstdio>
#include <cstdlib>
#include <cstdlib>
#include <vector>

#include "common.h"
#include "exact.cuh"
#include "index.h"
#include "kernels.h"
#include "search_common.cuh"
#include "pm_common.cuh"

#pragma clang fp contract(off)

namespace lh {

#ifndef LH_PM_BS
#define LH_PM_BS 512
#endif
#ifndef LH_PM_STATIC_LUT
#define LH_PM_STATIC_LUT 0
#endif
constexpr int PM_BS = LH_PM_BS;
constexpr int PM_CAP = PM_BS + 256;
// ... 30 lines not shown
__global__ __launch_bounds__(256) void pm_keys_kernel(const uint32_t *__restrict__ probes, int64_t npairs, int nprobes, int nlist,
                                                      uint32_t *__restrict__ keys) {
  const int64_t i = (int64_t)blockIdx.x * 256 + threadIdx.x;
  if (i >= npairs) return;
  keys[i] = probes[i] + ((i % nprobes) == 0 ? 0u : (uint32_t)nlist);
}

__global__ __launch_bounds__(256) void pm_item_table_kernel(const uint32_t *__restrict__ pair_starts, int nlist,
                                                            uint32_t *__restrict__ item_start) {
  __shared__ uint32_t wsum[4];
  __shared__ uint32_t carry_s;
  const int lane = threadIdx.x & 63, wave = threadIdx.x >> 6;
  if (threadIdx.x == 0) carry_s = 0;
  __syncthreads();
  for (int base = 0; base < nlist; base += 256) {
    const int i = base + threadIdx.x;
    const uint32_t v = i < nlist ? (pair_starts[i + 1] - pair_starts[i] + 1) / 2 : 0;
    uint32_t incl = v;
#pragma unroll
    for (int off = 1; off < 64; off <<= 1) {
      const uint32_t t = __shfl_up(incl, off, 64);
      if (lane >= off) incl += t;
    }
    if (lane == 63) wsum[wave] = incl;
    __syncthreads();
    uint32_t woff = 0;
    for (int w = 0; w < wave; ++w) woff += wsum[w];
    const uint32_t carry = carry_s;
    if (i < nlist) item_start[i] = carry + woff + incl - v;
    __syncthreads();
    if (threadIdx.x == 255) carry_s = carry + woff + incl;
    __syncthreads();
  }
  if (threadIdx.x == 0) item_start[nlist] = carry_s;
}

__global__ __launch_bounds__(256) void pm_item_desc_kernel(const uint32_t *__restrict__ item_start, const uint32_t *__restrict__ pair_starts,
                                                           const uint32_t *__restrict__ pair_idx, int nvp, int nlist, int nprobes, uint32_t max_items,
                                                           int4 *__restrict__ desc) {
  const uint32_t item = blockIdx.x * 256 + threadIdx.x;
  if (item >= max_items) return;
  int4 dsc = make_int4(-1, -1, -1, 0);
  if (item < item_start[nvp]) {
    int vp = (int)find_partition_dev(item_start, nvp, item);
    while (item_start[vp + 1] <= item) ++vp;
    const uint32_t g = item - item_start[vp];
    const uint32_t ps = pair_starts[vp], pe = pair_starts[vp + 1];
    const uint32_t i0 = ps + 2 * g;
    dsc.x = vp % nlist;
    dsc.y = (int)(pair_idx[i0] / (uint32_t)nprobes);
    dsc.z = i0 + 1 < pe ? (int)(pair_idx[i0 + 1] / (uint32_t)nprobes) : -1;
  }
  desc[item] = dsc;
}

template <int SD, int METRIC, int MU, int RPL, int CAP>
__device__ __forceinline__ void pm_scan_item(const PmArgs &p, const uint32_t item) {
  extern __shared__ __attribute__((aligned(16))) char smem[];
  constexpr int m = MU * 16;
  constexpr int Q = SD / 4;
  const int dpad = (p.d + 3) & ~3;
  float *r0 = reinterpret_cast<float *>(smem);
  float *r1 = r0 + dpad;
#if LH_PM_STATIC_LUT
  __shared__ __attribute__((aligned(16))) f2 lut2[m * 256];
  uint32_t *ck0 = reinterpret_cast<uint32_t *>(r1 + dpad);
#else
  f2 *lut2 = reinterpret_cast<f2 *>(r1 + dpad);
  uint32_t *ck0 = reinterpret_cast<uint32_t *>(lut2 + m * 256);
#endif
  uint32_t *cp0 = ck0 + CAP;
  uint32_t *ck1 = cp0 + CAP;
  uint32_t *cp1 = ck1 + CAP;
  uint32_t *sorted = cp1 + CAP;
  uint32_t *misc = sorted + PM_BS;
  __shared__ int s_part, s_q0, s_q1, s_valid;

  const int cb_c = threadIdx.x & 255, cb_half = threadIdx.x >> 8;
  constexpr int MH = m / (PM_BS / 256), MA = MH / 2;
  f4 cbA[MA][Q];
#pragma unroll
  for (int i = 0; i < MA; ++i) {
    const f4 *src = reinterpret_cast<const f4 *>(p.codebook + ((int64_t)(cb_half * MH + i) * 256 + cb_c) * SD);
#pragma unroll
    for (int u = 0; u < Q; ++u) cbA[i][u] = src[u];
  }

  if (threadIdx.x == 0) {
    const uint32_t it = p.loop ? item : item + (p.cls == 1 ? p.item_start[p.nlist] : 0u);
    const int valid = p.loop ? 1 : (it < p.item_start[(p.cls == 0 ? 1 : 2) * p.nlist]);
    int4 dsc = make_int4(0, -1, -1, 0);
    if (valid) dsc = p.desc[it];
    const int part = dsc.x, q0 = dsc.y, q1 = dsc.z;
    s_valid = valid; s_part = part; s_q0 = q0; s_q1 = q1;
    misc[0] = 0; misc[2] = 0; misc[5] = 0;
  }
  const long long pt0 = p.prof ? clock64() : 0;
  __syncthreads();
  if (!s_valid) return;
  const long long pt1 = p.prof ? clock64() : 0;
  const int part = s_part, q0 = s_q0, q1 = s_q1;
  const bool has1 = q1 >= 0;
  float qa_v = 0.0f, qb_v = 0.0f, cen_v = 0.0f;
  if ((int)threadIdx.x < p.d) {
    qa_v = p.q[(int64_t)q0 * p.d + threadIdx.x];
    qb_v = p.q[(int64_t)(has1 ? q1 : q0) * p.d + threadIdx.x];
// ... 365 lines not shown
static int ivfpq_scan_merge_q(lance_hip_ctx *ctx, const lance_hip_index *ix, const float *qs, uint32_t nq, const uint32_t *probes,
                              uint32_t nprobes, uint32_t keff, uint32_t k, bool do_refine, uint64_t *ids, float *dists,
                              uint64_t *cand_rid, uint32_t *cand_cnt, uint32_t *flags, const uint32_t *allow) {
  const int d = (int)ix->d, m = (int)ix->m, sd = d / m, nlist = (int)ix->nlist;
  const size_t npairs = (size_t)nq * nprobes;
  const uint32_t max_items2 = (uint32_t)(npairs / 2 + 2 * nlist + 2);
  const uint32_t max_items4 = (uint32_t)(npairs / 4 + nlist + 2);
  uint32_t *keys = ctx->scratch_t<uint32_t>("pm.keys", npairs);
  uint32_t *pair_starts = ctx->scratch_t<uint32_t>("pm.pair_starts", (size_t)2 * nlist + 1);
  uint32_t *pair_idx = ctx->scratch_t<uint32_t>("pm.pair_idx", npairs);
  uint32_t *item_start = ctx->scratch_t<uint32_t>("pm.item_start", (size_t)2 * nlist + 1);
  int4 *desc = ctx->scratch_t<int4>("pm.desc", max_items2);
  uint32_t *pair_starts0 = ctx->scratch_t<uint32_t>("q.pair_starts0", (size_t)nlist + 1);
  static const uint32_t dot_nb_env = getenv("LANCE_HIP_DOT_BOUND_LISTS") ? (uint32_t)std::max(1, atoi(getenv("LANCE_HIP_DOT_BOUND_LISTS"))) : 3u;
  static const uint32_t l2_nb_env = getenv("LANCE_HIP_BOUND_LISTS") ? (uint32_t)std::max(1, atoi(getenv("LANCE_HIP_BOUND_LISTS"))) : 1u;
  static const bool no_msbound_env = getenv("LANCE_HIP_NO_MSBOUND") != nullptr || getenv("LANCE_HIP_EXACT_BOUND") != nullptr;
  const uint32_t l2_nb = (!no_msbound_env && l2_nb_env > 1 && mscan_supported(ix, nq, nprobes) && qscan_pt_mode(ix) != 2) ? l2_nb_env : 1u;
  const uint32_t nb0 = std::min<uint32_t>(std::min<uint32_t>(ix->metric == LANCE_HIP_DOT ? dot_nb_env : l2_nb, 4u), nprobes);
  const uint32_t max_items0 = (uint32_t)((size_t)nq * nb0 / 2 + nlist + 2);
  uint32_t *pair_idx0 = ctx->scratch_t<uint32_t>("q.pair_idx0", (size_t)nq * nb0);
  uint32_t *item_start0 = ctx->scratch_t<uint32_t>("q.item_start0", (size_t)nlist + 1);
  int4 *desc0 = ctx->scratch_t<int4>("q.desc0", max_items0);
  uint32_t *item_start4 = ctx->scratch_t<uint32_t>("q.item_start4", (size_t)nlist + 1);
  int4 *desc4 = ctx->scratch_t<int4>("q.desc4", max_items4);
  uint32_t *tglobal = ctx->scratch_t<uint32_t>("pm.tglobal", (size_t)nq * 4);
  uint32_t *seg_cnt = ctx->scratch_t<uint32_t>("q.seg_cnt", npairs);
  uint32_t *seg_pos = ctx->scratch_t<uint32_t>("q.seg_pos", npairs * QSCAN_SEG_CAP);
  uint64_t pool_max = qscan_tiled_shape(m, sd) ? 65536 : 8192;
  while (pool_max > 8192 && (uint64_t)nq * pool_max * 8 > (1ull << 30)) pool_max /= 2;
  int pool_cap = (int)std::min<uint64_t>(pool_max, std::max<uint64_t>(512, (uint64_t)nprobes * (keff + 28)));
  pool_cap = (pool_cap + 255) & ~255;
  uint32_t *pool_key = ctx->scratch_t<uint32_t>("pm.pool_key", (size_t)nq * pool_cap);
  uint32_t *pool_pos = ctx->scratch_t<uint32_t>("pm.pool_pos", (size_t)nq * pool_cap);
  if (!keys || !pair_starts || !pair_idx || !item_start || !desc || !pair_starts0 || !pair_idx0 || !item_start0 || !desc0 || !item_start4 ||
      !desc4 || !tglobal || !seg_cnt || !seg_pos || !pool_key || !pool_pos)
    return LANCE_HIP_ENOMEM;
  uint32_t *pool_cnt = tglobal + nq, *tbound = tglobal + 2 * (size_t)nq, *qovf = tglobal + 3 * (size_t)nq;
  LH_CHECK_HIP(lh::memset_multi(ctx->stream, {{tglobal, 0xFF, (size_t)nq * 4}, {pool_cnt, 0, (size_t)nq * 4}}));
  PmArgs a;
  a.q = qs; a.probes = probes;
  a.centroids = ix->centroids; a.codebook = ix->codebook; a.part_offsets = ix->part_offsets; a.codes = ix->codes;
  a.d = d; a.m = m; a.nprobes = (int)nprobes; a.nlist = nlist; a.keff = (int)keff;
  const bool dot = ix->metric == LANCE_HIP_DOT;
  a.residual = dot ? 0 : 1;
  a.round_f16 = ix->dtype == LANCE_HIP_F16 ? 1 : 0;
  a.prof = nullptr;
  a.tglobal = tglobal; a.pool_key = pool_key; a.pool_pos = pool_pos; a.pool_cnt = pool_cnt; a.pool_cap = pool_cap; a.flags = flags;
  a.unbounded = 0; a.loop = 0; a.allow = allow;
  const bool tiled = qscan_tiled_shape(m, sd);
  static const bool exact_bound_env = getenv("LANCE_HIP_EXACT_BOUND") != nullptr;
  const bool exact_bound = exact_bound_env && !tiled && !dot;
  {
    ScopedTimer t(ctx, "pm_group");
    LH_TRY(qscan_nearest_keys(ctx, probes, nq, nprobes, keys, nb0));
    LH_TRY(stable_group(ctx, keys, (int64_t)nq * nb0, (int64_t)nq * nb0, nlist, 1, pair_starts0, pair_idx0, (int64_t)nq * nb0, nullptr));
    if (exact_bound) {
      hipLaunchKernelGGL(pm_item_table_kernel, dim3(1), dim3(256), 0, ctx->stream, pair_starts0, nlist, item_start0);
      hipLaunchKernelGGL(pm_item_desc_kernel, dim3((unsigned)cdiv(max_items0, 256)), dim3(256), 0, ctx->stream, item_start0, pair_starts0, pair_idx0,
                         nlist, nlist, 1, max_items0, desc0);
    }
  }
  if (exact_bound) {
    ScopedTimer t(ctx, "ivfpq_scan_c0");
    a.pair_starts = pair_starts0; a.pair_idx = pair_idx0; a.item_start = item_start0; a.desc = desc0;
    a.cls = 0; a.bound_pass = 1;
    const size_t lds = pm_lds_base(d, m) + (size_t)PM_CAP_BOUND * 16;
    const bool ok = launch_pm_sd<METRIC_L2>(ctx, a, sd, (unsigned)(nq / 2 + nlist + 1), lds);
    LH_REQUIRE(ok, "partition-major scan: unsupported shape (m=%d, sd=%d)", m, sd);
  } else if (!dot && qscan_pt_mode(ix) == 2) {
    ScopedTimer t(ctx, "ivfpq_scan_c0");
    LH_TRY(qbound_pt_launch(ctx, ix, qs, nq, nprobes, keff, probes, pair_starts0, pair_idx0, item_start0, desc0, (uint32_t)(nq / 4 + nlist + 2), tglobal,
                            allow));
  } else {
    ScopedTimer t(ctx, "ivfpq_scan_c0");
    int mb_rc = LH_NOT_TAKEN;
    if (mscan_supported(ix, nq, nprobes))
      mb_rc = msbound_launch(ctx, ix, qs, nq, keff, pair_starts0, pair_idx0, item_start0, desc0, (uint32_t)((size_t)nq * nb0 / 4 + nlist + 2), tglobal, allow, nb0);
    if (mb_rc < 0) return mb_rc;
    if (mb_rc == LH_NOT_TAKEN && dot) return LH_NOT_TAKEN;
    if (mb_rc == LH_NOT_TAKEN) LH_TRY(qbound_launch(ctx, ix, qs, nq, keff, pair_starts0, pair_idx0, item_start0, desc0, (uint32_t)(nq / 4 + nlist + 2), tglobal, allow));
  }
  {
    ScopedTimer t(ctx, "pm_group");
    LH_TRY(qscan_group(ctx, probes, nq, nprobes, nlist, tglobal, keys, tbound, pair_starts, pair_idx, item_start4, desc4, max_items4, 4, dot ? 1 : 0));
    hipLaunchKernelGGL(pm_item_table_kernel, dim3(1), dim3(256), 0, ctx->stream, pair_starts, 2 * nlist, item_start);
    hipLaunchKernelGGL(pm_item_desc_kernel, dim3((unsigned)cdiv(max_items2, 256)), dim3(256), 0, ctx->stream, item_start, pair_starts, pair_idx,
                       2 * nlist, nlist, (int)nprobes, max_items2, desc);
  }
  uint32_t *qslack = nullptr;
  float *seg_val = nullptr, *seg_scale = nullptr;
  int ms_rc = LH_NOT_TAKEN;
  if (mscan_supported(ix, nq, nprobes))
    ms_rc = mscan_launch(ctx, ix, qs, nq, nprobes, probes, pair_starts, pair_idx, tbound, seg_cnt, seg_pos, qovf, allow, &qslack, &seg_val, &seg_scale);
  if (ms_rc < 0) return ms_rc;
  if (ms_rc == LH_NOT_TAKEN && dot) return LH_NOT_TAKEN;
  if (ms_rc == LH_NOT_TAKEN) {
    qslack = nullptr; seg_val = nullptr; seg_scale = nullptr;
    LH_TRY(qscan_launch(ctx, ix, qs, nq, nprobes, pair_idx, item_start4, desc4, max_items4, tbound, seg_cnt, seg_pos, qovf, allow, probes));
  }
  static const bool q_stats = getenv("LANCE_HIP_Q_STATS") != nullptr;
  if (q_stats) {
    std::vector<uint32_t> sc(npairs), tb(nq);
    (void)hipMemcpyAsync(sc.data(), seg_cnt, npairs * 4, hipMemcpyDeviceToHost, ctx->stream);
    (void)hipMemcpyAsync(tb.data(), tbound, (size_t)nq * 4, hipMemcpyDeviceToHost, ctx->stream);
    (void)hipStreamSynchronize(ctx->stream);
    uint64_t tot = 0, ovf = 0, mx = 0, nb = 0, r0 = 0;
    for (size_t i = 0; i < npairs; ++i) { tot += std::min<uint32_t>(sc[i], QSCAN_SEG_CAP); ovf += sc[i] > (uint32_t)QSCAN_SEG_CAP; mx = std::max<uint64_t>(mx, sc[i]); if (i % nprobes == 0) r0 += sc[i]; }
    for (uint32_t i = 0; i < nq; ++i) nb += tb[i] == 0xFFFFFFFFu;
    fprintf(stderr, "[qscan] nq=%u nprobes=%u keff=%u survivors/query %.1f (nearest partition %.1f) max segment %llu overflowed segments %llu class-B queries %llu\n",
            nq, nprobes, keff, (double)tot / nq, (double)r0 / nq, (unsigned long long)mx, (unsigned long long)ovf, (unsigned long long)nb);
  }
  if (tiled) {
    ScopedTimer t(ctx, "ivfpq_scan_cb");
    LH_TRY(qscan_classb_to_rescan(ctx, tbound, nq, nprobes, seg_cnt, qovf));
  } else {
    ScopedTimer t(ctx, "ivfpq_scan_cb");
    a.pair_starts = pair_starts; a.pair_idx = pair_idx; a.item_start = item_start; a.desc = desc;
    a.cls = 1; a.bound_pass = 0; a.unbounded = 1; a.loop = 1;
    const size_t lds = pm_lds_base(d, m) + (size_t)PM_CAP * 16;
    const unsigned grid = (unsigned)std::min<uint64_t>((uint64_t)ctx->num_cus * 3, (uint64_t)max_items2);
    const bool ok = dot ? launch_pm_sd<METRIC_DOT>(ctx, a, sd, grid, lds) : launch_pm_sd<METRIC_L2>(ctx, a, sd, grid, lds);
    LH_REQUIRE(ok, "partition-major scan: unsupported shape (m=%d, sd=%d)", m, sd);
  }
  {
    SelectOut o;
    o.keff = (int)keff; o.k = (int)k; o.refine = do_refine ? 1 : 0;
    o.out_ids = ids; o.out_dists = dists; o.cand_rid = cand_rid; o.cand_cnt = cand_cnt; o.flags = flags;
    o.part_offsets = ix->part_offsets; o.nlist = nlist;
    ScopedTimer t(ctx, "ivfpq_merge");
    LH_TRY(qmerge_launch(ctx, ix, qs, nq, probes, nprobes, tbound, tglobal, seg_cnt, seg_pos, qovf, pool_key, pool_pos, pool_cnt, pool_cap, o, allow, qslack, seg_val, seg_scale));
  }
  LH_CHECK_HIP(hipGetLastError());
  return LANCE_HIP_OK;
}

int ivfpq_scan_merge_pm(lance_hip_ctx *ctx, const lance_hip_index *ix, const float *qs, uint32_t nq, const uint32_t *probes,
                        uint32_t nprobes, uint32_t keff, uint32_t k, bool do_refine, uint64_t *ids, float *dists,
                        uint64_t *cand_rid, uint32_t *cand_cnt, uint32_t *flags, const uint32_t *allow) {
  const int d = (int)ix->d, m = (int)ix->m, sd = d / m, nlist = (int)ix->nlist;
  const int scan_metric = ix->metric == LANCE_HIP_COSINE ? LANCE_HIP_L2 : ix->metric;
  if (!pm_nobound() && qscan_supported(ix, nq, nprobes)) {
    const int rc = ivfpq_scan_merge_q(ctx, ix, qs, nq, probes, nprobes, keff, k, do_refine, ids, dists, cand_rid, cand_cnt, flags, allow);
    if (rc != LH_NOT_TAKEN) return rc;
  }
  const size_t npairs = (size_t)nq * nprobes;
  uint32_t *pair_starts = ctx->scratch_t<uint32_t>("pm.pair_starts", (size_t)2 * nlist + 1);
  uint32_t *pair_idx = ctx->scratch_t<uint32_t>("pm.pair_idx", npairs);
  uint32_t *item_start = ctx->scratch_t<uint32_t>("pm.item_start", (size_t)2 * nlist + 1);
  uint32_t *tglobal = ctx->scratch_t<uint32_t>("pm.tglobal", (size_t)nq * 2);
  int pool_cap = (int)std::min<uint64_t>(8192, std::max<uint64_t>(512, (uint64_t)nprobes * (keff + 28)));
  pool_cap = (pool_cap + 255) & ~255;
  uint32_t *pool_key = ctx->scratch_t<uint32_t>("pm.pool_key", (size_t)nq * pool_cap);
  uint32_t *pool_pos = ctx->scratch_t<uint32_t>("pm.pool_pos", (size_t)nq * pool_cap);
  if (!pair_starts || !pair_idx || !item_start || !tglobal || !pool_key || !pool_pos) return LANCE_HIP_ENOMEM;
  uint32_t *pool_cnt = tglobal + nq;
  LH_CHECK_HIP(lh::memset_multi(ctx->stream, {{tglobal, 0xFF, (size_t)nq * 4}, {pool_cnt, 0, (size_t)nq * 4}}));
  uint32_t *keys = ctx->scratch_t<uint32_t>("pm.keys", npairs);
  const uint32_t max_items = (uint32_t)(npairs / 2 + 2 * nlist + 2);
  int4 *desc = ctx->scratch_t<int4>("pm.desc", max_items);
  if (!keys || !desc) return LANCE_HIP_ENOMEM;
  {
    ScopedTimer t(ctx, "pm_group");
    hipLaunchKernelGGL(pm_keys_kernel, dim3((unsigned)cdiv(npairs, 256)), dim3(256), 0, ctx->stream, probes, (int64_t)npairs, (int)nprobes,
                       nlist, keys);
    LH_TRY(stable_group(ctx, keys, (int64_t)npairs, (int64_t)npairs, 2 * nlist, 1, pair_starts, pair_idx, (int64_t)npairs, nullptr));
    hipLaunchKernelGGL(pm_item_table_kernel, dim3(1), dim3(256), 0, ctx->stream, pair_starts, 2 * nlist, item_start);
    hipLaunchKernelGGL(pm_item_desc_kernel, dim3((unsigned)cdiv(max_items, 256)), dim3(256), 0, ctx->stream, item_start, pair_starts, pair_idx,
                       2 * nlist, nlist, (int)nprobes, max_items, desc);
  }
  PmArgs a;
  a.q = qs; a.probes = probes; a.pair_starts = pair_starts; a.pair_idx = pair_idx; a.item_start = item_start;
  a.centroids = ix->centroids; a.codebook = ix->codebook; a.part_offsets = ix->part_offsets; a.codes = ix->codes;
  a.d = d; a.m = m; a.nprobes = (int)nprobes; a.nlist = nlist; a.keff = (int)keff;
  a.residual = scan_metric == LANCE_HIP_L2 ? 1 : 0;
  a.round_f16 = ix->dtype == LANCE_HIP_F16 ? 1 : 0;
  a.desc = desc;
  a.unbounded = 0; a.loop = 0; a.allow = allow;
  a.prof = nullptr;
  static const bool pm_prof = getenv("LANCE_HIP_PM_PROF") != nullptr;
  if (pm_prof) {
    a.prof = ctx->scratch_t<unsigned long long>("pm.prof", 8);
    if (a.prof) (void)lh::memset_async(a.prof, 0, 64, ctx->stream);
  }
  a.tglobal = tglobal; a.pool_key = pool_key; a.pool_pos = pool_pos; a.pool_cnt = pool_cnt; a.pool_cap = pool_cap; a.flags = flags;
  const size_t lds_base = pm_lds_base(d, m);
  {
    const bool nobound = pm_nobound();
    for (int pass = 0; pass < 2; ++pass) {
      if (nobound && pass == 1 && nprobes == 1) break;
      ScopedTimer t(ctx, pass == 0 ? "ivfpq_scan_c0" : "ivfpq_scan_c1");
      a.cls = pass == 0 ? 0 : (nobound ? 1 : 2);
      a.bound_pass = (pass == 0 && !nobound) ? 1 : 0;
      const size_t lds = lds_base + (size_t)(a.bound_pass ? PM_CAP_BOUND : PM_CAP) * 16;
      const size_t cpairs = a.cls == 0 ? (size_t)nq : (a.cls == 1 ? (size_t)nq * (nprobes - 1) : (size_t)nq * nprobes);
      const unsigned grid = (unsigned)(cpairs / 2 + (a.cls == 2 ? 2 : 1) * nlist + 1);
      bool ok = false;
      if (scan_metric == LANCE_HIP_DOT) {
        if (sd == 4) ok = launch_pm_mu<4, METRIC_DOT>(ctx, a, grid, lds);
        else if (sd == 8) ok = launch_pm_mu<8, METRIC_DOT>(ctx, a, grid, lds);
        else if (sd == 16) ok = launch_pm_mu<16, METRIC_DOT>(ctx, a, grid, lds);
      } else {
        if (sd == 4) ok = launch_pm_mu<4, METRIC_L2>(ctx, a, grid, lds);
        else if (sd == 8) ok = launch_pm_mu<8, METRIC_L2>(ctx, a, grid, lds);
        else if (sd == 16) ok = launch_pm_mu<16, METRIC_L2>(ctx, a, grid, lds);
      }
      LH_REQUIRE(ok, "partition-major scan: unsupported shape (m=%d, sd=%d)", m, sd);
      if (a.prof && pass == 1) {
        unsigned long long h[8];
        (void)hipMemcpyAsync(h, a.prof, 64, hipMemcpyDeviceToHost, ctx->stream);
        (void)hipStreamSynchronize(ctx->stream);
        if (h[5]) fprintf(stderr, "[pm prof] items=%llu clocks/item: desc %.0f | q,centroid,residual %.0f | LUT %.0f | scan %.0f | publish %.0f\n", h[5],
                          (double)h[0] / h[5], (double)h[1] / h[5], (double)h[2] / h[5], (double)h[3] / h[5], (double)h[4] / h[5]);
        (void)lh::memset_async(a.prof, 0, 64, ctx->stream);
      }
    }
  }
  {
    SelectOut o;
    o.keff = (int)keff; o.k = (int)k; o.refine = do_refine ? 1 : 0;
    o.out_ids = ids; o.out_dists = dists; o.cand_rid = cand_rid; o.cand_cnt = cand_cnt; o.flags = flags;
    o.part_offsets = ix->part_offsets; o.nlist = nlist;
// ... 9 lines not shown
```

### lance_amd/csrc/search_q.hip

```cpp
#include <algorithm>
#include <cstdio>
#include <cstdlib>

#include "common.h"
#include "exact.cuh"
#include "index.h"
#include "kernels.h"
#include "search_common.cuh"
#include "pm_common.cuh"
#include "q_common.cuh"

#pragma clang fp contract(off)

namespace lh {

__global__ __launch_bounds__(256) void q_tclass_keys_kernel(const uint32_t *__restrict__ probes, int64_t npairs, int nprobes, int nlist,
                                                            const uint32_t *__restrict__ tglobal, uint32_t *__restrict__ keys,
                                                            uint32_t *__restrict__ tbound, int dot) {
  const int64_t i = (int64_t)blockIdx.x * 256 + threadIdx.x;
  if (i >= npairs) return;
  const int64_t q = i / nprobes;
  const uint32_t T = tglobal[q];
  const bool usable = T > (dot ? 0x007FFFFFu : 0x80000000u) && T < 0xFF800000u;
  keys[i] = probes[i] + (usable ? 0u : (uint32_t)nlist);
  if (i % nprobes == 0) tbound[q] = usable ? T : 0xFFFFFFFFu;
}

__global__ __launch_bounds__(256) void q_nearest_keys_kernel(const uint32_t *__restrict__ probes, int nq, int nprobes, int nb, uint32_t *__restrict__ keys) {
  const int i = blockIdx.x * 256 + threadIdx.x;
  if (i < nq * nb) keys[i] = probes[(int64_t)(i / nb) * nprobes + (i % nb)];
}

__global__ __launch_bounds__(256) void q_item_table_kernel(const uint32_t *__restrict__ pair_starts, int nvp, int G, uint32_t *__restrict__ item_start) {
  __shared__ uint32_t wsum[4];
  __shared__ uint32_t carry_s;
  const int lane = threadIdx.x & 63, wave = threadIdx.x >> 6;
  if (threadIdx.x == 0) carry_s = 0;
  __syncthreads();
  for (int base = 0; base < nvp; base += 256) {
    const int i = base + threadIdx.x;
    const uint32_t v = i < nvp ? (pair_starts[i + 1] - pair_starts[i] + G - 1) / G : 0;
    uint32_t incl = v;
#pragma unroll
    for (int off = 1; off < 64; off <<= 1) {
      const uint32_t t = __shfl_up(incl, off, 64);
      if (lane >= off) incl += t;
    }
    if (lane == 63) wsum[wave] = incl;
    __syncthreads();
    uint32_t woff = 0;
    for (int w = 0; w < wave; ++w) woff += wsum[w];
    const uint32_t carry = carry_s;
    if (i < nvp) item_start[i] = carry + woff + incl - v;
    __syncthreads();
    if (threadIdx.x == 255) carry_s = carry + woff + incl;
    __syncthreads();
  }
  if (threadIdx.x == 0) item_start[nvp] = carry_s;
}

__global__ __launch_bounds__(256) void q_item_desc_kernel(const uint32_t *__restrict__ item_start, const uint32_t *__restrict__ pair_starts,
                                                          int nvp, int G, uint32_t max_items, int4 *__restrict__ desc) {
  const uint32_t item = blockIdx.x * 256 + threadIdx.x;
  if (item >= max_items) return;
  int4 dsc = make_int4(-1, 0, 0, 0);
  if (item < item_start[nvp]) {
    int vp = (int)find_partition_dev(item_start, nvp, item);
    while (item_start[vp + 1] <= item) ++vp;
    const uint32_t g = item - item_start[vp];
    const uint32_t ps = pair_starts[vp], pe = pair_starts[vp + 1];
    const uint32_t i0 = ps + (uint32_t)G * g;
    dsc.x = vp;
    dsc.y = (int)i0;
    dsc.z = (int)min((uint32_t)G, pe - i0);
  }
  desc[item] = dsc;
}

__global__ __launch_bounds__(256) void q_residual_kernel(const float *__restrict__ q, const uint32_t *__restrict__ pair_idx,
                                                         const uint32_t *__restrict__ item_start, const int4 *__restrict__ desc,
                                                         const float *__restrict__ centroids, int d, int nlist, int pdiv, int round_f16,
                                                         f4 *__restrict__ rq) {
  const uint32_t item = blockIdx.x * 4u + (threadIdx.x >> 6);
  if (item >= item_start[nlist]) return;
  const int lane = threadIdx.x & 63;
  const int4 dsc = desc[item];
  const int part = dsc.x, i0 = dsc.y, cnt = dsc.z;
  uint32_t qj[Q_G];
#pragma unroll
  for (int j = 0; j < Q_G; ++j) qj[j] = pair_idx[i0 + (j < cnt ? j : 0)] / (uint32_t)pdiv;
  for (int dim = lane; dim < d; dim += 64) {
    const float cen = centroids[(int64_t)part * d + dim];
    f4 r4;
#pragma unroll
    for (int j = 0; j < Q_G; ++j) {
      float v = q[(int64_t)qj[j] * d + dim] - cen;
      if (round_f16) v = __half2float(__float2half_rn(v));
      r4[j] = -v;
    }
    rq[(int64_t)item * d + dim] = r4;
  }
}

template <int SD, int MU>
__global__ __launch_bounds__(Q_BS, (MU == 1 ? (SD <= 8 ? Q_WAVES : 6) : 4)) void ivfpq_qscan_kernel(QscanArgs p) {
  extern __shared__ __attribute__((aligned(16))) char smem[];
  constexpr int M = MU * 16;
  constexpr uint32_t CAPE = 65535u / M;
  constexpr uint32_t SE = CAPE - CAPE / 32;
  constexpr uint32_t LIM = SE + M + 2;
  static_assert(LIM < CAPE - 1, "a saturated entry must put the row above the limit");
  __shared__ __attribute__((aligned(16))) uint2 lutq[M * 256];
  uint32_t *cand = reinterpret_cast<uint32_t *>(smem);
  uint32_t *misc = cand + 4 * Q_CAP;
  float *sc = reinterpret_cast<float *>(misc + 4);
  uint16_t *csum = reinterpret_cast<uint16_t *>(sc + 4);

  const uint32_t item = blockIdx.x;
  if (item >= p.item_start[p.nlist]) return;
  {
    const int4 dsc = p.desc[item];
    const int part = dsc.x, i0 = dsc.y, cnt = dsc.z;
// ... 849 lines not shown
        for (int i = threadIdx.x; i < o.keff; i += BS) o.cand_rid[(int64_t)q * o.keff + i] = i < c1 ? a.row_ids[cpos[i]] : ~0ull;
        if (threadIdx.x == 0) o.cand_cnt[q] = (uint32_t)c1;
        return;
      }
    }
  }
  for (int iter = 0; iter < 8 && (int)misc[0] > SCAN_LCAP; ++iter) tighten_bs<BS, CAP>(b, o.keff, sorted, &misc[2]);
  __syncthreads();
  int c = min((int)misc[0], CAP);
  if (c > SCAN_LCAP || misc[3]) {
    if (threadIdx.x == 0) atomicOr(&o.flags[q], FLAG_OVERFLOW);
    c = min(c, SCAN_LCAP);
  }
  for (int i = threadIdx.x; i < SCAN_LCAP; i += BS) {
    if (i < c) { skey[i] = ckey[i]; spos[i] = cpos[i]; rid[i] = a.row_ids[cpos[i]]; }
    else { skey[i] = 0xFFFFFFFFu; spos[i] = 0; rid[i] = ~0ull; }
  }
  __syncthreads();
  int Pq = 64;
  while (Pq < c) Pq <<= 1;
  bitonic_sort_kr<BS>(skey, rid, spos, Pq);
  QM_DBG_RETURN(a, 5);
  select_and_emit<BS>(o, q, skey, rid, spos, c, &s_amb);
}

bool qscan_supported(const lance_hip_index *ix, uint32_t nq, uint32_t nprobes) {
  static const bool off = getenv("LANCE_HIP_NO_QSCAN") != nullptr;
  if (off || !ix->model_finite) return false;
  const int scan_metric = ix->metric == LANCE_HIP_COSINE ? LANCE_HIP_L2 : ix->metric;
  if (scan_metric == LANCE_HIP_DOT) { if (!mscan_dot_ready(ix, nq, nprobes)) return false; }
  else if (scan_metric != LANCE_HIP_L2) return false;
  {
    const int m = (int)ix->m, sd = (int)(ix->d / ix->m);
    if (!((m == 16 || m == 32) && (sd == 4 || sd == 8 || sd == 16)) && !qscan_tiled_shape(m, sd)) return false;
  }
  if ((uint64_t)nq * nprobes * Q_CAP * 4 > (2ull << 30)) return false;
  const bool needs_rq = !qscan_pt_enabled(ix) && !mscan_batch_shape(ix, nq, nprobes);
  if (needs_rq && ((uint64_t)nq * nprobes / Q_G + ix->nlist + 1) * ix->d * 16 > (2ull << 30)) return false;
  return true;
}

size_t qscan_lds_bytes(int d, int m) {
  (void)d; (void)m;
  return (size_t)4 * Q_CAP * 4 + 8 * 4 + (size_t)4 * Q_CAP * 2;
}

int qscan_group(lance_hip_ctx *ctx, const uint32_t *probes, uint32_t nq, uint32_t nprobes, int nlist, const uint32_t *tglobal,
                uint32_t *keys, uint32_t *tbound, uint32_t *pair_starts, uint32_t *pair_idx, uint32_t *item_start4, int4 *desc4,
                uint32_t max_items4, int G, int dot) {
  const size_t npairs = (size_t)nq * nprobes;
  hipLaunchKernelGGL(q_tclass_keys_kernel, dim3((unsigned)cdiv(npairs, 256)), dim3(256), 0, ctx->stream, probes, (int64_t)npairs, (int)nprobes,
                     nlist, tglobal, keys, tbound, dot);
  LH_TRY(stable_group(ctx, keys, (int64_t)npairs, (int64_t)npairs, 2 * nlist, 1, pair_starts, pair_idx, (int64_t)npairs, nullptr));
  hipLaunchKernelGGL(q_item_table_kernel, dim3(1), dim3(256), 0, ctx->stream, pair_starts, nlist, G, item_start4);
  hipLaunchKernelGGL(q_item_desc_kernel, dim3((unsigned)cdiv(max_items4, 256)), dim3(256), 0, ctx->stream, item_start4, pair_starts, nlist, G,
                     max_items4, desc4);
  return LANCE_HIP_OK;
}

int qscan_item_tables(lance_hip_ctx *ctx, const uint32_t *pair_starts, int nlist, int G, uint32_t *item_start, int4 *desc, uint32_t max_items) {
  hipLaunchKernelGGL(q_item_table_kernel, dim3(1), dim3(256), 0, ctx->stream, pair_starts, nlist, G, item_start);
  hipLaunchKernelGGL(q_item_desc_kernel, dim3((unsigned)cdiv(max_items, 256)), dim3(256), 0, ctx->stream, item_start, pair_starts, nlist, G, max_items, desc);
  return LANCE_HIP_OK;
}

int qscan_nearest_keys(lance_hip_ctx *ctx, const uint32_t *probes, uint32_t nq, uint32_t nprobes, uint32_t *keys, uint32_t nb) {
  hipLaunchKernelGGL(q_nearest_keys_kernel, dim3((unsigned)cdiv((uint64_t)nq * nb, 256)), dim3(256), 0, ctx->stream, probes, (int)nq, (int)nprobes, (int)nb, keys);
  return LANCE_HIP_OK;
}

template <int SD>
static bool launch_qscan_sd(lance_hip_ctx *ctx, const QscanArgs &a, int m, unsigned grid, size_t lds) {
  if (m == 16) { hipLaunchKernelGGL((ivfpq_qscan_kernel<SD, 1>), dim3(grid), dim3(Q_BS), lds, ctx->stream, a); return true; }
  if (m == 32) { hipLaunchKernelGGL((ivfpq_qscan_kernel<SD, 2>), dim3(grid), dim3(Q_BS), lds, ctx->stream, a); return true; }
  return false;
}

int qscan_launch(lance_hip_ctx *ctx, const lance_hip_index *ix, const float *qs, uint32_t nq, uint32_t nprobes, const uint32_t *pair_idx,
                 const uint32_t *item_start4, const int4 *desc4, uint32_t max_items4, const uint32_t *tbound, uint32_t *seg_cnt,
                 uint32_t *seg_pos, uint32_t *qovf, const uint32_t *allow, const uint32_t *probes) {
  const int d = (int)ix->d, m = (int)ix->m, sd = d / m;
  const bool pt = probes != nullptr && qscan_pt_enabled(ix);
  f4 *rq = pt ? nullptr : reinterpret_cast<f4 *>(ctx->scratch_t<float>("qscan.rq", (size_t)max_items4 * d * 4));
  if (!pt && !rq) return LANCE_HIP_ENOMEM;
  {
    ScopedTimer t(ctx, "q_residual");
    if (!pt)
      hipLaunchKernelGGL(q_residual_kernel, dim3((unsigned)cdiv(max_items4, 4)), dim3(256), 0, ctx->stream, qs, pair_idx, item_start4, desc4,
                         ix->centroids, d, (int)ix->nlist, (int)nprobes, ix->dtype == LANCE_HIP_F16 ? 1 : 0, rq);
    LH_CHECK_HIP(lh::memset_async(seg_cnt, 0, (size_t)nq * nprobes * 4, ctx->stream));
    LH_CHECK_HIP(lh::memset_async(qovf, 0, (size_t)nq * 4, ctx->stream));
  }
  ScopedTimer t(ctx, "ivfpq_scan_c1");
  QscanArgs a;
  a.rq = rq; a.pair_idx = pair_idx; a.item_start = item_start4; a.desc = desc4;
  a.centroids = ix->centroids; a.codebook = ix->codebook; a.part_offsets = ix->part_offsets; a.codes = ix->codes;
  a.d = d; a.nprobes = (int)nprobes; a.nlist = (int)ix->nlist; a.round_f16 = ix->dtype == LANCE_HIP_F16 ? 1 : 0;
  a.tbound = tbound; a.seg_cnt = seg_cnt; a.seg_pos = seg_pos; a.qovf = qovf; a.allow = allow;
  a.seg_sum = ctx->scratch_t<uint16_t>("q.seg_sum", (size_t)nq * nprobes * Q_CAP);
  a.ovf = ctx->scratch_t<uint32_t>("q.ovf", (size_t)nq * nprobes + 1);
  if (!a.seg_sum || !a.ovf) return LANCE_HIP_ENOMEM;
  LH_CHECK_HIP(lh::memset_async(a.ovf, 0, 4, ctx->stream));
  const size_t lds = qscan_lds_bytes(d, m);
  const unsigned grid = max_items4;
  bool ok = false;
#ifdef LH_QT_PROF
  static const bool qt_prof = getenv("LANCE_HIP_QT_PROF") != nullptr;
  if (qt_prof && qscan_tiled_shape(m, sd)) {
    a.prof = ctx->scratch_t<unsigned long long>("qt.prof", 8);
    if (a.prof) (void)lh::memset_async(a.prof, 0, 64, ctx->stream);
  }
#endif
  if (pt) { LH_TRY(qscan_pt_launch(ctx, ix, a, qs, nq, probes, grid)); ok = true; }
// ... 12 lines not shown
#endif
  return LANCE_HIP_OK;
}

template <int SD>
static bool launch_qbound_sd(lance_hip_ctx *ctx, const QboundArgs &a, int m, unsigned grid, size_t lds) {
  if (m == 16) { hipLaunchKernelGGL((ivfpq_qbound_kernel<SD, 1>), dim3(grid), dim3(Q_BS), lds, ctx->stream, a); return true; }
  if (m == 32) { hipLaunchKernelGGL((ivfpq_qbound_kernel<SD, 2>), dim3(grid), dim3(Q_BS), lds, ctx->stream, a); return true; }
  return false;
}

__global__ __launch_bounds__(256) void q_codebook_mean_kernel(const float *__restrict__ codebook, int sd, int d, float *__restrict__ out) {
  __shared__ float part[4];
  const int mm = blockIdx.x, c = threadIdx.x, lane = c & 63, wave = c >> 6;
  const float *cw = codebook + ((int64_t)mm * 256 + c) * sd;
  float sq = 0.0f;
  for (int e = 0; e <= sd; ++e) {
    float v;
    if (e < sd) { v = cw[e]; sq += v * v; } else v = sq;
#pragma unroll
    for (int o = 32; o > 0; o >>= 1) v += __shfl_xor(v, o, 64);
    __syncthreads();
    if (lane == 0) part[wave] = v;
    __syncthreads();
    if (c == 0) {
      const float tot = (part[0] + part[1] + part[2] + part[3]) * (1.0f / 256.0f);
      if (e < sd) out[mm * sd + e] = tot; else atomicAdd(&out[d], tot);
    }
  }
}

__global__ __launch_bounds__(256) void q_model_finite_kernel(const float *__restrict__ a, int64_t na, const float *__restrict__ b, int64_t nb,
                                                             uint32_t *__restrict__ flag) {
  const int64_t i = (int64_t)blockIdx.x * 256 + threadIdx.x;
  bool bad = false;
  if (i < na) bad = !isfinite(a[i]);
  else if (i < na + nb) bad = !isfinite(b[i - na]);
  if (__any(bad) && (threadIdx.x & 63) == 0) atomicOr(flag, 1u);
}

int qscan_index_constants(lance_hip_ctx *ctx, lance_hip_index *ix) {
  const int d = (int)ix->d, m = (int)ix->m;
  if (!ix->cb_mean) LH_CHECK_HIP(hipMalloc(reinterpret_cast<void **>(&ix->cb_mean), (size_t)(d + 2) * 4));
  LH_CHECK_HIP(lh::memset_async(ix->cb_mean, 0, (size_t)(d + 2) * 4, ctx->stream));
  hipLaunchKernelGGL(q_codebook_mean_kernel, dim3((unsigned)m), dim3(256), 0, ctx->stream, ix->codebook, d / m, d, ix->cb_mean);
  const int64_t nc = (int64_t)ix->nlist * d, ncb = (int64_t)m * 256 * (d / m);
  hipLaunchKernelGGL(q_model_finite_kernel, dim3((unsigned)cdiv((uint64_t)(nc + ncb), 256)), dim3(256), 0, ctx->stream, ix->centroids, nc, ix->codebook,
                     ncb, reinterpret_cast<uint32_t *>(ix->cb_mean + d + 1));
  LH_CHECK_HIP(hipGetLastError());
  return LANCE_HIP_OK;
}

int qscan_items(lance_hip_ctx *ctx, const uint32_t *pair_starts, int nvp, int G, uint32_t *item_start, int4 *desc, uint32_t max_items) {
  hipLaunchKernelGGL(q_item_table_kernel, dim3(1), dim3(256), 0, ctx->stream, pair_starts, nvp, G, item_start);
  hipLaunchKernelGGL(q_item_desc_kernel, dim3((unsigned)cdiv(max_items, 256)), dim3(256), 0, ctx->stream, item_start, pair_starts, nvp, G, max_items, desc);
  LH_CHECK_HIP(hipGetLastError());
  return LANCE_HIP_OK;
}

int qbound_launch(lance_hip_ctx *ctx, const lance_hip_index *ix, const float *qs, uint32_t nq, uint32_t keff, const uint32_t *pair_starts0,
                  const uint32_t *pair_idx0, uint32_t *item_start, int4 *desc, uint32_t max_items, uint32_t *tglobal, const uint32_t *allow) {
  const int d = (int)ix->d, m = (int)ix->m, sd = d / m, nlist = (int)ix->nlist;
  hipLaunchKernelGGL(q_item_table_kernel, dim3(1), dim3(256), 0, ctx->stream, pair_starts0, nlist, Q_G, item_start);
  hipLaunchKernelGGL(q_item_desc_kernel, dim3((unsigned)cdiv(max_items, 256)), dim3(256), 0, ctx->stream, item_start, pair_starts0, nlist, Q_G,
                     max_items, desc);
  f4 *rq = reinterpret_cast<f4 *>(ctx->scratch_t<float>("qbound.rq", (size_t)max_items * d * 4));
  if (!rq) return LANCE_HIP_ENOMEM;
  hipLaunchKernelGGL(q_residual_kernel, dim3((unsigned)cdiv(max_items, 4)), dim3(256), 0, ctx->stream, qs, pair_idx0, item_start, desc, ix->centroids, d,
                     nlist, 1, ix->dtype == LANCE_HIP_F16 ? 1 : 0, rq);
  QboundArgs a;
  a.rq = rq; a.pair_idx = pair_idx0; a.item_start = item_start; a.desc = desc;
  a.centroids = ix->centroids; a.codebook = ix->codebook; a.part_offsets = ix->part_offsets; a.codes = ix->codes;
  a.d = d; a.nlist = nlist; a.keff = (int)keff; a.round_f16 = ix->dtype == LANCE_HIP_F16 ? 1 : 0;
  a.tglobal = tglobal; a.allow = allow;
  LH_REQUIRE(ix->cb_mean, "integer bound pass: the index carries no codebook means (8-bit PQ only)");
  a.cb_mean = ix->cb_mean;
  const size_t lds = (size_t)4 * QB_BINS * 4 + 8 * 4;
  bool ok = false;
  if (qscan_tiled_shape(m, sd)) ok = qbound_tiled_launch(ctx, a, m, sd, max_items);
  else if (sd == 4) ok = launch_qbound_sd<4>(ctx, a, m, max_items, lds);
  else if (sd == 8) ok = launch_qbound_sd<8>(ctx, a, m, max_items, lds);
  else if (sd == 16) ok = launch_qbound_sd<16>(ctx, a, m, max_items, lds);
  LH_REQUIRE(ok, "integer bound pass: unsupported shape (m=%d, sd=%d)", m, sd);
  (void)nq;
  return LANCE_HIP_OK;
}

template <int SD, int MU, bool DOT = false>
static void launch_qmerge_mu(lance_hip_ctx *ctx, const QmergeArgs &a, unsigned nq, int bs) {
  const int dpad = (a.d + 3) & ~3;
  const size_t lds_rescan = (size_t)dpad * 4 + (size_t)MU * 16 * 256 * 4;
  const unsigned rgrid = (unsigned)std::min<uint64_t>((uint64_t)nq * a.nprobes, (uint64_t)ctx->num_cus);
  hipLaunchKernelGGL((ivfpq_qrescan_kernel<SD, MU, 1024, DOT>), dim3(rgrid), dim3(1024), lds_rescan, ctx->stream, a);
  const size_t lds = std::max((size_t)std::min<int>(a.qm_g, a.nprobes) * dpad * 4, (size_t)SCAN_LCAP * 16);
  static const bool v1 = getenv("LANCE_HIP_QMERGE_V1") != nullptr;
  if (!v1 && a.nprobes <= a.qm_g) {
    if (bs == 256) hipLaunchKernelGGL((ivfpq_qmerge1g_kernel<SD, MU, 256, DOT>), dim3(nq), dim3(256), lds, ctx->stream, a);
    else hipLaunchKernelGGL((ivfpq_qmerge1g_kernel<SD, MU, 128, DOT>), dim3(nq), dim3(128), lds, ctx->stream, a);
    return;
  }
  if (bs == 256) hipLaunchKernelGGL((ivfpq_qmerge_kernel<SD, MU, 256, DOT>), dim3(nq), dim3(256), lds, ctx->stream, a);
  else hipLaunchKernelGGL((ivfpq_qmerge_kernel<SD, MU, 128, DOT>), dim3(nq), dim3(128), lds, ctx->stream, a);
}

int qmerge_launch(lance_hip_ctx *ctx, const lance_hip_index *ix, const float *qs, uint32_t nq, const uint32_t *probes, uint32_t nprobes,
                  const uint32_t *tbound, uint32_t *tglobal, const uint32_t *seg_cnt, const uint32_t *seg_pos, const uint32_t *qovf,
                  uint32_t *pool_key, uint32_t *pool_pos, uint32_t *pool_cnt, int pool_cap, const SelectOut &o, const uint32_t *allow,
                  const uint32_t *qslack, const float *seg_val, const float *seg_scale) {
  const int d = (int)ix->d, m = (int)ix->m, sd = d / m;
  QmergeArgs a;
  a.qslack = qslack; a.seg_val = seg_val; a.seg_pv = reinterpret_cast<const uint2 *>(seg_val); a.seg_scale = reinterpret_cast<const f2 *>(seg_scale);
#ifdef LH_TIMING_EXPERIMENTS
  {
    static const int dbg = [] {
      const int v = getenv("LANCE_HIP_QM_DBG") ? atoi(getenv("LANCE_HIP_QM_DBG")) : 0;
      if (v) fprintf(stderr, "lance_hip: LANCE_HIP_QM_DBG=%d -- timing experiment, search RESULTS ARE WRONG\n", v);
      return v;
    }();
// ... 66 lines not shown
```

Before: 25.23 million queries/s.

## Fuse coarse selection, single-block small grouping, and merged item-table kernels

Adds a fused coarse-assignment kernel that computes query-centroid dot products with split-bf16 MFMA in LDS and runs the top-nprobes selection in the same launch, for nlist below 1024. It also adds a single-workgroup stable grouping kernel for small problems that reads probe ids directly, which skips the separate key-building pass and the multi-block histogram. Item-table and descriptor building are merged into one kernel that keeps the start table in LDS. The aim is to cut kernel launches and global round trips in the search pipeline. The cost is more LDS pressure and a fixed one-block limit on the grouping kernel.

```diff
diff --git a/lance_amd/csrc/ctx.cpp b/lance_amd/csrc/ctx.cpp
--- a/lance_amd/csrc/ctx.cpp
+++ b/lance_amd/csrc/ctx.cpp
@@ -219,6 +219,12 @@
     if (launches) *launches = it == ctx->stage_counts.end() ? 0 : it->second;
     return LANCE_HIP_OK;
   }
+  if (strncmp(kernel, "scratch:", 8) == 0) {
+    auto it = ctx->slots.find(kernel + 8);
+    if (ms_total) *ms_total = it == ctx->slots.end() ? 0.0 : (double)reinterpret_cast<uintptr_t>(it->second.first);
+    if (launches) *launches = it == ctx->slots.end() ? 0 : (uint64_t)it->second.second;
+    return LANCE_HIP_OK;
+  }
   auto &t = ctx->timers[kernel];
   for (auto &ev : t.pending) {
     float ms = 0.f;
diff --git a/lance_amd/csrc/group.hip b/lance_amd/csrc/group.hip
--- a/lance_amd/csrc/group.hip
+++ b/lance_amd/csrc/group.hip
@@ -1,3 +1,5 @@
+#include <cstdlib>
+
 #include "common.h"
 #include "kernels.h"
 
@@ -203,6 +205,94 @@
     }
     __syncthreads();
   }
+}
+
+constexpr int GROUP_SMALL_WAVES = 16, GROUP_SMALL_MAX_N = 16384, GROUP_SMALL_MAX_K = 1024;
+
+__global__ __launch_bounds__(1024) void group_small_kernel(const uint32_t *__restrict__ src, int n, int key_div, int key_stride, int k, int kbits,
+                                                           uint32_t *__restrict__ starts, uint32_t *__restrict__ sorted_rows) {
+  extern __shared__ uint32_t cnt[];
+  __shared__ uint32_t wsum[GROUP_SMALL_WAVES];
+  constexpr int W = GROUP_SMALL_WAVES;
+  const int lane = threadIdx.x & 63, wave = threadIdx.x >> 6;
+  const int total = k * W;
+  for (int i = threadIdx.x; i < total; i += 1024) cnt[i] = 0u;
+  __syncthreads();
+  const int nchunks = (n + 63) / 64, per = (nchunks + W - 1) / W;
+  const int c_begin = min(nchunks, wave * per), c_end = min(nchunks, c_begin + per);
+  auto key_at = [&](int r) -> uint32_t {
+    if (r >= n) return LANCE_HIP_NONE;
+    return key_div ? src[(int64_t)(r / key_div) * key_stride + (r % key_div)] : src[r];
+  };
+  for (int c = c_begin; c < c_end; c += 8) {
+    uint32_t key[8];
+#pragma unroll
+    for (int u = 0; u < 8; ++u) key[u] = c + u < c_end ? key_at((c + u) * 64 + lane) : LANCE_HIP_NONE;
+#pragma unroll
+    for (int u = 0; u < 8; ++u)
+      if (key[u] < (uint32_t)k) atomicAdd(&cnt[key[u] * W + wave], 1u);
+  }
+  __syncthreads();
+  {
+    const int run = (total + 1023) / 1024;
+    const int lo = min(total, (int)threadIdx.x * run), hi = min(total, lo + run);
+    uint32_t s = 0;
+    for (int i = lo; i < hi; ++i) s += cnt[i];
+    uint32_t incl = s;
+#pragma unroll
+    for (int off = 1; off < 64; off <<= 1) {
+      const uint32_t t = __shfl_up(incl, off, 64);
+      if (lane >= off) incl += t;
+    }
+    if (lane == 63) wsum[wave] = incl;
+    __syncthreads();
+    uint32_t run_off = incl - s;
+    for (int w = 0; w < wave; ++w) run_off += wsum[w];
+    for (int i = lo; i < hi; ++i) { const uint32_t v = cnt[i]; cnt[i] = run_off; run_off += v; }
+    if (threadIdx.x == 1023) starts[k] = run_off;
+  }
+  __syncthreads();
+  for (int c = threadIdx.x; c < k; c += 1024) starts[c] = cnt[c * W];
+  __syncthreads();
+  const uint64_t below = lane == 0 ? 0ull : (~0ull >> (64 - lane));
+  for (int c = c_begin; c < c_end; c += 8) {
+    uint32_t key[8];
+#pragma unroll
+    for (int u = 0; u < 8; ++u) key[u] = c + u < c_end ? key_at((c + u) * 64 + lane) : LANCE_HIP_NONE;
+#pragma unroll
+    for (int u = 0; u < 8; ++u) {
+      if (c + u >= c_end) break;
+      const bool valid = key[u] < (uint32_t)k;
+      uint64_t mask = __ballot(valid);
+      for (int bit = 0; bit < kbits; ++bit) {
+        const bool one = (key[u] >> bit) & 1u;
+        const uint64_t bal = __ballot(one);
+        mask &= one ? bal : ~bal;
+      }
+      if (valid) {
+        const uint32_t base = cnt[key[u] * W + wave];
+        const uint32_t rank = (uint32_t)__popcll(mask & below);
+        sorted_rows[base + rank] = (uint32_t)((c + u) * 64 + lane);
+        if (rank == 0) cnt[key[u] * W + wave] = base + (uint32_t)__popcll(mask);
+      }
+      __builtin_amdgcn_wave_barrier();
+    }
+  }
+}
+
+bool stable_group_small_ok(int64_t n, int k) {
+  static const bool off = getenv("LANCE_HIP_NO_GROUP_SMALL") != nullptr;
+  return !off && n <= GROUP_SMALL_MAX_N && k > 0 && k <= GROUP_SMALL_MAX_K;
+}
+
+int stable_group_small(lance_hip_ctx *ctx, const uint32_t *src, int64_t n, int key_div, int64_t key_stride, int k, uint32_t *starts, uint32_t *sorted_rows) {
+  LH_REQUIRE(stable_group_small_ok(n, k), "stable_group_small: n=%lld k=%d not supported", (long long)n, k);
+  int kbits = 0;
+  while ((1 << kbits) < k) ++kbits;
+  hipLaunchKernelGGL(group_small_kernel, dim3(1), dim3(1024), (size_t)k * GROUP_SMALL_WAVES * 4, ctx->stream, src, (int)n, key_div, (int)key_stride, k, kbits,
+                     starts, sorted_rows);
+  LH_CHECK_HIP(hipGetLastError());
+  return LANCE_HIP_OK;
 }
 
 __global__ __launch_bounds__(256) void group_digit_lo_kernel(const uint32_t *__restrict__ ids, int64_t n, int k, uint32_t *__restrict__ out) {
@@ -258,6 +348,7 @@
     LH_REQUIRE(batches == 1 && active == nullptr, "stable_group: more than 16384 keys only for a single problem");
     return stable_group_wide(ctx, ids, n, k, starts, sorted_rows);
   }
+  if (batches == 1 && active == nullptr && stable_group_small_ok(n, k)) return stable_group_small(ctx, ids, n, 0, 0, k, starts, sorted_rows);
   const int nblocks = (int)cdiv(n > 0 ? n : 1, GROUP_ROWS_PER_BLOCK);
   uint32_t *blockhist = ctx->scratch_t<uint32_t>("group.blockhist", (size_t)batches * k * nblocks);
   uint32_t *totals = ctx->scratch_t<uint32_t>("group.totals", (size_t)batches * k);
diff --git a/lance_amd/csrc/kernels.h b/lance_amd/csrc/kernels.h
--- a/lance_amd/csrc/kernels.h
+++ b/lance_amd/csrc/kernels.h
@@ -102,12 +102,17 @@
 size_t xform_coarse_planes_elems(uint32_t nlist, int d);
 int xform_coarse_planes(lance_hip_ctx *ctx, int metric, const float *cent, uint32_t nlist, int d, uint16_t *cpl, uint32_t *maxbits );
 bool coarse_groups_shape(int d, uint32_t nlist);
+bool coarse_fused_shape(int d, uint32_t nlist);
+size_t coarse_fused_planes_elems(uint32_t nlist, int d);
+int coarse_fused_planes(lance_hip_ctx *ctx, const float *cent, uint32_t nlist, int d, uint16_t *cpl, uint32_t *maxbits );
 bool mfma_assign_supported(const PairwiseArgs &p, int d, int batches);
 int launch_assign_mfma(lance_hip_ctx *ctx, const PairwiseArgs &p, int d, int metric);
 int launch_dist_matrix(lance_hip_ctx *ctx, const PairwiseArgs &p, int d, int metric, int batches);
 
 int stable_group(lance_hip_ctx *ctx, const uint32_t *ids, int64_t n, int64_t id_stride, int k, int batches,
                  uint32_t *starts, uint32_t *sorted_rows, int64_t out_stride, const uint8_t *active);
+bool stable_group_small_ok(int64_t n, int k);
+int stable_group_small(lance_hip_ctx *ctx, const uint32_t *src, int64_t n, int key_div, int64_t key_stride, int k, uint32_t *starts, uint32_t *sorted_rows);
 
 int kmeans_train_batched(lance_hip_ctx *ctx, int metric, const float *x, int64_t n, int64_t ldx, int x_batch_off, int d,
                          int k, int B, uint32_t max_iters, double tol, float balance_factor_scaled, bool have_init,
diff --git a/lance_amd/csrc/mfma_assign.hip b/lance_amd/csrc/mfma_assign.hip
--- a/lance_amd/csrc/mfma_assign.hip
+++ b/lance_amd/csrc/mfma_assign.hip
@@ -874,26 +874,13 @@
   return finish_metric<METRIC>(s + tot);
 }
 
-template <int METRIC, bool GROUPS = false>
-__global__ __launch_bounds__(256) void coarse_select_kernel(float *__restrict__ sur, const float *__restrict__ e2, const float *__restrict__ q,
-                                                            const float *__restrict__ cent, int nq, int nlist, int d, int nprobes,
-                                                            uint32_t *__restrict__ part_ids, float *__restrict__ dists,
-                                                            uint32_t *__restrict__ n_exact_rows, const float *__restrict__ gkey = nullptr,
-                                                            const float *__restrict__ gsec = nullptr, int ng = 0) {
-  extern __shared__ __attribute__((aligned(16))) char smem[];
-  const int lane = threadIdx.x & 63, wave = threadIdx.x >> 6, grp = lane >> 4;
-  const int qi = blockIdx.x * 4 + wave;
-  if (qi >= nq) return;
-  const int dpad = (d + 3) & ~3;
+template <int METRIC, bool GROUPS>
+__device__ __forceinline__ void cs_select_row(float *row, const float *gk, int ng, const float E2, const float *wrow, unsigned long long *ck,
+                                              uint32_t *cl, const float *__restrict__ cent, int qi, int nlist, int d, int nprobes,
+                                              uint32_t *__restrict__ part_ids, float *__restrict__ dists, uint32_t *__restrict__ n_exact_rows,
+                                              int lane) {
+  const int grp = lane >> 4;
   constexpr int CAP = GROUPS ? CS_CAP_G : CS_CAP;
-  float *wrow = reinterpret_cast<float *>(smem) + (size_t)wave * dpad;
-  unsigned long long *ck = reinterpret_cast<unsigned long long *>(smem + (size_t)4 * dpad * 4) + (size_t)wave * CAP;
-  uint32_t *cl = reinterpret_cast<uint32_t *>(smem + (size_t)4 * dpad * 4 + (size_t)4 * CAP * 8) + (size_t)wave * CAP;
-  const float *qv = q + (int64_t)qi * d;
-  for (int e = lane; e < d; e += 64) wrow[e] = qv[e];
-  float *row = sur + (int64_t)qi * nlist;
-  const float E2 = GROUPS ? e2[qi] * 1.0625f : e2[qi];
-  const float *gk = GROUPS ? gkey + (int64_t)qi * 2 * ng : nullptr;
   float m0 = INFINITY, m1 = INFINITY, m2 = INFINITY, m3 = INFINITY;
   bool bad = !(E2 < INFINITY) || !(E2 > 7.888609052210118e-31f);
   auto ins4 = [&](float v) {
@@ -1067,6 +1054,136 @@
   }
 }
 
+template <int METRIC, bool GROUPS = false>
+__global__ __launch_bounds__(256) void coarse_select_kernel(float *__restrict__ sur, const float *__restrict__ e2, const float *__restrict__ q,
+                                                            const float *__restrict__ cent, int nq, int nlist, int d, int nprobes,
+                                                            uint32_t *__restrict__ part_ids, float *__restrict__ dists,
+                                                            uint32_t *__restrict__ n_exact_rows, const float *__restrict__ gkey = nullptr,
+                                                            const float *__restrict__ gsec = nullptr, int ng = 0) {
+  extern __shared__ __attribute__((aligned(16))) char smem[];
+  const int lane = threadIdx.x & 63, wave = threadIdx.x >> 6;
+  const int qi = blockIdx.x * 4 + wave;
+  if (qi >= nq) return;
+  const int dpad = (d + 3) & ~3;
+  constexpr int CAP = GROUPS ? CS_CAP_G : CS_CAP;
+  float *wrow = reinterpret_cast<float *>(smem) + (size_t)wave * dpad;
+  unsigned long long *ck = reinterpret_cast<unsigned long long *>(smem + (size_t)4 * dpad * 4) + (size_t)wave * CAP;
+  uint32_t *cl = reinterpret_cast<uint32_t *>(smem + (size_t)4 * dpad * 4 + (size_t)4 * CAP * 8) + (size_t)wave * CAP;
+  const float *qv = q + (int64_t)qi * d;
+  for (int e = lane; e < d; e += 64) wrow[e] = qv[e];
+  float *row = sur + (int64_t)qi * nlist;
+  const float E2 = GROUPS ? e2[qi] * 1.0625f : e2[qi];
+  const float *gk = GROUPS ? gkey + (int64_t)qi * 2 * ng : nullptr;
+  cs_select_row<METRIC, GROUPS>(row, gk, ng, E2, wrow, ck, cl, cent, qi, nlist, d, nprobes, part_ids, dists, n_exact_rows, lane);
+}
+
+struct CfArgs {
+  const float *q;
+  const float *cent;
+  const uint16_t *chi, *clo;
+  const float *cn;
+  const uint32_t *maxbits;
+  uint32_t *n_exact;
+  uint32_t *part_ids;
+  float *dists;
+  int nq, nlist, nprobes, qt;
+};
+
+template <int KS, int METRIC>
+__global__ __launch_bounds__(512, 4) void coarse_fused_kernel(CfArgs p) {
+  extern __shared__ __attribute__((aligned(16))) char smem[];
+  constexpr int D = KS * 16;
+  constexpr int XS = D + 4;
+  const int lane = threadIdx.x & 63, wave = threadIdx.x >> 6, nw = blockDim.x >> 6;
+  const int j = lane & 31, g = lane >> 5;
+  const int nblk = (p.nlist + 31) >> 5, SS = nblk * 32 + 4;
+  const int QT = p.qt;
+  constexpr int PS = D + 8;
+  float *xs = reinterpret_cast<float *>(smem);
+  uint16_t *xph = reinterpret_cast<uint16_t *>(xs + (size_t)QT * XS);
+  uint16_t *xpl = xph + (size_t)QT * PS;
+  float *sur = reinterpret_cast<float *>(xpl + (size_t)QT * PS);
+  unsigned long long *ck = reinterpret_cast<unsigned long long *>(sur + (size_t)QT * SS) + (size_t)wave * CS_CAP;
+  uint32_t *cl = reinterpret_cast<uint32_t *>(reinterpret_cast<unsigned long long *>(sur + (size_t)QT * SS) + (size_t)nw * CS_CAP) + (size_t)wave * CS_CAP;
+  float *e2s = reinterpret_cast<float *>(reinterpret_cast<uint32_t *>(reinterpret_cast<unsigned long long *>(sur + (size_t)QT * SS) + (size_t)nw * CS_CAP) + (size_t)nw * CS_CAP);
+  const int q0 = blockIdx.x * QT;
+
+  for (int idx = threadIdx.x; idx < QT * (D / 4); idx += blockDim.x) {
+    const int r = idx / (D / 4), c4 = idx - r * (D / 4);
+    f4 v = {0.0f, 0.0f, 0.0f, 0.0f};
+    if (q0 + r < p.nq) v = *reinterpret_cast<const f4 *>(p.q + (int64_t)(q0 + r) * D + 4 * c4);
+    *reinterpret_cast<f4 *>(&xs[r * XS + 4 * c4]) = v;
+  }
+  __syncthreads();
+  for (int idx = threadIdx.x; idx < QT * (D / 8); idx += blockDim.x) {
+    const int r = idx / (D / 8), c8 = idx - r * (D / 8);
+    const f4 a = *reinterpret_cast<const f4 *>(&xs[r * XS + 8 * c8]), b = *reinterpret_cast<const f4 *>(&xs[r * XS + 8 * c8 + 4]);
+    const float v[8] = {a.x, a.y, a.z, a.w, b.x, b.y, b.z, b.w};
+    bf16x8 h, l;
+#pragma unroll
+    for (int e = 0; e < 8; ++e) {
+      const uint32_t hb = bf16_rne_bits(v[e]);
+      h[e] = (short)hb; l[e] = (short)bf16_rne_bits(v[e] - bf16_bits_to_float(hb));
+    }
+    *reinterpret_cast<bf16x8 *>(xph + r * PS + 8 * c8) = h;
+    *reinterpret_cast<bf16x8 *>(xpl + r * PS + 8 * c8) = l;
+  }
+  const int jr = min(j, QT - 1);
+  const float *xr = xs + jr * XS + g * 8;
+  if (wave == 0) {
+    float xn2 = 0.0f;
+#pragma unroll
+    for (int s = 0; s < KS; ++s) {
+      const f4 a = *reinterpret_cast<const f4 *>(xr + s * 16), b = *reinterpret_cast<const f4 *>(xr + s * 16 + 4);
+      const float v[8] = {a.x, a.y, a.z, a.w, b.x, b.y, b.z, b.w};
+#pragma unroll
+      for (int e = 0; e < 8; ++e) xn2 += v[e] * v[e];
+    }
+    xn2 += __shfl_xor(xn2, 32, 64);
+    const float cmax2 = __uint_as_float(p.maxbits[0]), bmax = __uint_as_float(p.maxbits[1]);
+    if (g == 0) e2s[j] = 2.0f * 0.0001220703125f * (xn2 + cmax2 + bmax) + (METRIC == METRIC_DOT ? 4.7683716e-7f : 0.0f);
+  }
+  __syncthreads();
+
+  for (int b = wave; b < nblk; b += nw) {
+    const int cr = min(b * 32 + j, p.nlist - 1);
+    const uint16_t *hi = p.chi + (int64_t)cr * D + g * 8, *lo = p.clo + (int64_t)cr * D + g * 8;
+    f32x16 acc;
+#pragma unroll
+    for (int v = 0; v < 16; ++v) acc[v] = 0.0f;
+#pragma unroll
+    for (int s = 0; s < KS; ++s) {
+      const bf16x8 ah = *reinterpret_cast<const bf16x8 *>(hi + s * 16), al = *reinterpret_cast<const bf16x8 *>(lo + s * 16);
+      const bf16x8 xh = *reinterpret_cast<const bf16x8 *>(xph + jr * PS + s * 16 + g * 8), xl = *reinterpret_cast<const bf16x8 *>(xpl + jr * PS + s * 16 + g * 8);
+      acc = __builtin_amdgcn_mfma_f32_32x32x16_bf16(ah, xh, acc, 0, 0, 0);
+      acc = __builtin_amdgcn_mfma_f32_32x32x16_bf16(ah, xl, acc, 0, 0, 0);
+      acc = __builtin_amdgcn_mfma_f32_32x32x16_bf16(al, xh, acc, 0, 0, 0);
+    }
+#pragma unroll
+    for (int vq = 0; vq < 4; ++vq) {
+      const int c0 = b * 32 + 8 * vq + 4 * g;
+      f4 o;
+#pragma unroll
+      for (int e = 0; e < 4; ++e) {
+        const float dot = acc[vq * 4 + e];
+        const float cn = c0 + e < p.nlist ? p.cn[c0 + e] : 0.0f;
+        float v = METRIC == METRIC_DOT ? -dot : __builtin_fmaf(-2.0f, dot, cn);
+        v += 0.0f;
+        o[e] = v;
+      }
+      if (j < QT) *reinterpret_cast<f4 *>(&sur[j * SS + c0]) = o;
+    }
+  }
+  __syncthreads();
+
+  for (int r = wave; r < QT; r += nw) {
+    const int qi = q0 + r;
+    if (qi >= p.nq) break;
+    cs_select_row<METRIC, false>(sur + r * SS, nullptr, 0, e2s[r], xs + r * XS, ck, cl, p.cent, qi, p.nlist, D, p.nprobes, p.part_ids, p.dists, p.n_exact, lane);
+    __builtin_amdgcn_wave_barrier();
+  }
+}
+
 bool coarse_mfma_supported(int metric, int d, uint32_t nq, uint32_t nlist, uint32_t nprobes, bool lanes32, const float *q, const float *cent) {
   static const char *env = getenv("LANCE_HIP_MFMA_COARSE");
   static const bool off = env && env[0] == '0', force = env && env[0] == '1';
@@ -1102,6 +1219,45 @@
 bool coarse_groups_shape(int d, uint32_t nlist) {
   static const bool ma = getenv("LANCE_HIP_COARSE_GROUPS_MA") != nullptr;
   return !ma && d <= 128 && d % 16 == 0 && coarse_groups_from() > 0 && nlist >= (uint32_t)std::max(coarse_groups_from(), 256);
+}
+
+bool coarse_fused_shape(int d, uint32_t nlist) {
+  static const bool off = getenv("LANCE_HIP_NO_COARSE_FUSED") != nullptr;
+  return !off && d >= 16 && d <= 128 && d % 16 == 0 && nlist >= 32 && nlist < 1024 && !coarse_groups_shape(d, nlist);
+}
+size_t coarse_fused_planes_elems(uint32_t nlist, int d) { return (size_t)2 * nlist * d + (size_t)2 * nlist; }
+int coarse_fused_planes(lance_hip_ctx *ctx, const float *cent, uint32_t nlist, int d, uint16_t *cpl, uint32_t *maxbits) {
+  const size_t kd = (size_t)nlist * d;
+  hipLaunchKernelGGL(ma_prep_kernel, dim3(nlist), dim3(64), 0, ctx->stream, cent, (int)nlist, d, d, nullptr, cpl, cpl + kd, reinterpret_cast<float *>(cpl + 2 * kd),
+                     maxbits, nullptr);
+  LH_CHECK_HIP(hipGetLastError());
+  return LANCE_HIP_OK;
+}
+
+template <int KS>
+static void coarse_fused_launch(lance_hip_ctx *ctx, CfArgs a, int metric) {
+  constexpr int D = KS * 16;
+  const int nblk = (a.nlist + 31) / 32, ss = nblk * 32 + 4;
+  int nw = 8, qt = 8;
+  auto lds_of = [&](int qt_, int nw_) { return (size_t)qt_ * (D + 4 + ss) * 4 + (size_t)qt_ * (D + 8) * 4 + (size_t)nw_ * CS_CAP * 12 + 32 * 4; };
+  {
+    uint64_t best = ~0ull;
+    for (int nw_ = 8; nw_ >= 4; --nw_)
+      for (int r = 1; r <= 4 && nw_ * r <= 32; ++r) {
+        const int qt_ = nw_ * r;
+        const size_t l = lds_of(qt_, nw_);
+        if (l > (size_t)80 * 1024) break;
+        const uint64_t resident = std::min<uint64_t>(32 / nw_, ((size_t)160 * 1024) / l);
+        const uint64_t per_cu = cdiv(cdiv((uint64_t)a.nq, (uint64_t)qt_), (uint64_t)ctx->num_cus);
+        const uint64_t cost = per_cu * qt_ * (per_cu > resident ? 2 : 1) * 8 + r;
+        if (cost < best) { best = cost; qt = qt_; nw = nw_; }
+      }
+  }
+  const size_t lds = lds_of(qt, nw);
+  a.qt = qt;
+  const dim3 grid((unsigned)cdiv((uint64_t)a.nq, (uint64_t)qt)), block((unsigned)nw * 64);
+  if (metric == METRIC_DOT) hipLaunchKernelGGL((coarse_fused_kernel<KS, METRIC_DOT>), grid, block, lds, ctx->stream, a);
+  else hipLaunchKernelGGL((coarse_fused_kernel<KS, METRIC_L2>), grid, block, lds, ctx->stream, a);
 }
 
 int find_partitions_mfma(lance_hip_ctx *ctx, int metric, const float *q, uint32_t nq, int d, const float *cent, uint32_t nlist, uint32_t nprobes,
@@ -1124,8 +1280,32 @@
     if (!gkey) return LANCE_HIP_ENOMEM;
   }
   LH_CHECK_HIP(lh::memset_async(maxbits, 0, 16, ctx->stream));
+  const bool fused = coarse_fused_shape(d, nlist);
+  if (fused) {
+    ScopedTimer t(ctx, "dist_matrix");
+    ctx->count_stage("coarse_fused");
+    CfArgs f;
+    f.q = q; f.cent = cent; f.nq = (int)nq; f.nlist = (int)nlist; f.nprobes = (int)nprobes; f.part_ids = part_ids; f.dists = dists; f.n_exact = maxbits + 2;
+    if (cpl_ready && maxbits_ready) {
+      f.chi = cpl_ready; f.clo = cpl_ready + kd; f.cn = reinterpret_cast<const float *>(cpl_ready + 2 * kd); f.maxbits = maxbits_ready;
+    } else {
+      hipLaunchKernelGGL(ma_prep_kernel, dim3(nlist), dim3(64), 0, ctx->stream, cent, (int)nlist, d, dp, nullptr, chi, clo, cn, maxbits, nullptr);
+      f.chi = chi; f.clo = clo; f.cn = cn; f.maxbits = maxbits;
+    }
+    switch (d / 16) {
+      case 1: coarse_fused_launch<1>(ctx, f, metric); break;
+      case 2: coarse_fused_launch<2>(ctx, f, metric); break;
+      case 3: coarse_fused_launch<3>(ctx, f, metric); break;
+      case 4: coarse_fused_launch<4>(ctx, f, metric); break;
+      case 5: coarse_fused_launch<5>(ctx, f, metric); break;
+      case 6: coarse_fused_launch<6>(ctx, f, metric); break;
+      case 7: coarse_fused_launch<7>(ctx, f, metric); break;
+      default: coarse_fused_launch<8>(ctx, f, metric); break;
+    }
+  }
   static const bool groups_ma = getenv("LANCE_HIP_COARSE_GROUPS_MA") != nullptr;
-  if (groups && !groups_ma) {
+  if (fused) {
+  } else if (groups && !groups_ma) {
     ScopedTimer t(ctx, "dist_matrix");
     LH_TRY(launch_xform_sweep_groups(ctx, metric, q, nq, d, cent, nlist, maxbits, gkey, ng, e2, cpl_ready, maxbits_ready));
   } else {
@@ -1165,7 +1345,7 @@
       }
     }
   }
-  {
+  if (!fused) {
     ScopedTimer t(ctx, "select_probes");
     const int dpad = (d + 3) & ~3;
     const int cap = groups ? CS_CAP_G : CS_CAP;
diff --git a/lance_amd/csrc/search.hip b/lance_amd/csrc/search.hip
--- a/lance_amd/csrc/search.hip
+++ b/lance_amd/csrc/search.hip
@@ -927,12 +927,15 @@
   std::lock_guard<std::mutex> lk(ix->lazy_mu);
   if (ix->cq || ctx->capturing) return LANCE_HIP_OK;
   auto *cq = new lance_hip_index::CqConst();
-  bool ok = hipMalloc(reinterpret_cast<void **>(&cq->cpl), xform_coarse_planes_elems(ix->nlist, (int)ix->d) * 2) == hipSuccess;
+  const bool fused = coarse_fused_shape((int)ix->d, ix->nlist);
+  const size_t elems = fused ? coarse_fused_planes_elems(ix->nlist, (int)ix->d) : xform_coarse_planes_elems(ix->nlist, (int)ix->d);
+  bool ok = hipMalloc(reinterpret_cast<void **>(&cq->cpl), elems * 2) == hipSuccess;
   ok = ok && hipMalloc(reinterpret_cast<void **>(&cq->maxbits), 16) == hipSuccess;
   auto drop = [&]() { if (cq->cpl) (void)hipFree(cq->cpl); if (cq->maxbits) (void)hipFree(cq->maxbits); delete cq; };
   if (!ok) { (void)hipGetLastError(); drop(); return LANCE_HIP_OK; }
   if (lh::memset_async(cq->maxbits, 0, 16, ctx->stream) != hipSuccess ||
-      xform_coarse_planes(ctx, scan_metric, ix->centroids, ix->nlist, (int)ix->d, cq->cpl, cq->maxbits) != LANCE_HIP_OK ||
+      (fused ? coarse_fused_planes(ctx, ix->centroids, ix->nlist, (int)ix->d, cq->cpl, cq->maxbits)
+             : xform_coarse_planes(ctx, scan_metric, ix->centroids, ix->nlist, (int)ix->d, cq->cpl, cq->maxbits)) != LANCE_HIP_OK ||
       hipStreamSynchronize(ctx->stream) != hipSuccess) {
     drop();
     set_error("find_partitions: building the centroid planes of the index failed");
@@ -1360,7 +1363,7 @@
   if (coarse_mfma_supported(scan_metric, d, nq, (uint32_t)nlist, nprobes, coarse_l32, qs, ix->centroids)) {
     const uint16_t *cpl = nullptr;
     const uint32_t *cmb = nullptr;
-    if (coarse_groups_shape(d, (uint32_t)nlist)) {
+    if (coarse_groups_shape(d, (uint32_t)nlist) || coarse_fused_shape(d, (uint32_t)nlist)) {
       LH_TRY(coarse_planes_prepare(ctx, ix, scan_metric));
       if (ix->cq) { cpl = ix->cq->cpl; cmb = ix->cq->maxbits; }
     }
@@ -1520,7 +1523,7 @@
   LH_REQUIRE(ctx && idx, "index_prewarm: NULL argument");
   LH_CHECK_HIP(hipSetDevice(ctx->device));
   if (idx->m > 0 && idx->nbits == 8) LH_TRY(mscan_prewarm(ctx, idx));
-  if (coarse_groups_shape((int)idx->d, idx->nlist) && (reinterpret_cast<uintptr_t>(idx->centroids) & 15) == 0)
+  if ((coarse_groups_shape((int)idx->d, idx->nlist) || coarse_fused_shape((int)idx->d, idx->nlist)) && (reinterpret_cast<uintptr_t>(idx->centroids) & 15) == 0)
     LH_TRY(coarse_planes_prepare(ctx, idx, idx->metric == LANCE_HIP_COSINE ? LANCE_HIP_L2 : idx->metric));
   (void)raw_compact_prepare(ctx, idx);
   LH_CHECK_HIP(hipStreamSynchronize(ctx->stream));
diff --git a/lance_amd/csrc/search_common.cuh b/lance_amd/csrc/search_common.cuh
--- a/lance_amd/csrc/search_common.cuh
+++ b/lance_amd/csrc/search_common.cuh
@@ -23,6 +23,37 @@
     if (offs[mid] <= slot) lo = mid; else hi = mid;
   }
   return (uint32_t)lo;
+}
+
+constexpr int ITEMS_MAX_NVP = 2048;
+__device__ __forceinline__ void item_table_to_lds(const uint32_t *__restrict__ pair_starts, int nvp, int G, uint32_t *s_start, uint32_t *s_misc ,
+                                                  uint32_t *__restrict__ item_start) {
+  const int lane = threadIdx.x & 63, wave = threadIdx.x >> 6;
+  if (threadIdx.x == 0) s_misc[4] = 0;
+  __syncthreads();
+  for (int base = 0; base < nvp; base += 256) {
+    const int i = base + threadIdx.x;
+    const uint32_t v = i < nvp ? (pair_starts[i + 1] - pair_starts[i] + G - 1) / G : 0;
+    uint32_t incl = v;
+#pragma unroll
+    for (int off = 1; off < 64; off <<= 1) {
+      const uint32_t t = __shfl_up(incl, off, 64);
+      if (lane >= off) incl += t;
+    }
+    if (lane == 63) s_misc[wave] = incl;
+    __syncthreads();
+    uint32_t woff = 0;
+    for (int w = 0; w < wave; ++w) woff += s_misc[w];
+    const uint32_t carry = s_misc[4];
+    if (i < nvp) s_start[i] = carry + woff + incl - v;
+    __syncthreads();
+    if (threadIdx.x == 255) s_misc[4] = carry + woff + incl;
+    __syncthreads();
+  }
+  if (threadIdx.x == 0) s_start[nvp] = s_misc[4];
+  __syncthreads();
+  if (blockIdx.x == 0)
+    for (int i = threadIdx.x; i <= nvp; i += 256) item_start[i] = s_start[i];
 }
 
 template <int BS = 256>
diff --git a/lance_amd/csrc/search_ms.hip b/lance_amd/csrc/search_ms.hip
--- a/lance_amd/csrc/search_ms.hip
+++ b/lance_amd/csrc/search_ms.hip
@@ -288,6 +288,63 @@
     u.gs = gs + pb * sp.blk; u.qp = min(sp.blk, qp - pb * sp.blk); u.pad0 = u.pad1 = 0u;
     slices[s0 + t] = u;
     order[atomicAdd(&cls_cursor[ms_work_class(u.row_count, u.qp, cls_rows)], 1u)] = s0 + t;
+  }
+}
+
+constexpr int MS_SLICES_MAX_NLIST = 1024;
+__global__ __launch_bounds__(1024) void ms_slices_kernel(const uint32_t *__restrict__ pair_starts, const uint32_t *__restrict__ part_offsets, int nlist,
+                                                         uint32_t rs_rows, uint32_t rs2_rows, uint32_t cls_rows, uint32_t *__restrict__ slice_start,
+                                                         uint32_t *__restrict__ slice_ctr, MsSlice *__restrict__ slices, uint32_t *__restrict__ order) {
+  __shared__ uint32_t s_start[MS_SLICES_MAX_NLIST + 1], s_off[MS_SLICES_MAX_NLIST], s_np[MS_SLICES_MAX_NLIST], s_gs[MS_SLICES_MAX_NLIST], s_qp[MS_SLICES_MAX_NLIST];
+  __shared__ uint32_t wsum[16], hist[32], cur[32];
+  const int lane = threadIdx.x & 63, wave = threadIdx.x >> 6, i = threadIdx.x;
+  if (i == 0) slice_ctr[0] = 0u;
+  if (i < 32) hist[i] = 0u;
+  __syncthreads();
+  uint32_t v = 0;
+  if (i < nlist) {
+    const uint32_t gs = pair_starts[i], qp = pair_starts[i + 1] - gs, off = part_offsets[i], np = part_offsets[i + 1] - off;
+    s_off[i] = off; s_np[i] = np; s_gs[i] = gs; s_qp[i] = qp;
+    const MsSplit sp = ms_split(qp, np, rs_rows, rs2_rows);
+    v = sp.npb * sp.nrs;
+    for (uint32_t pb = 0; pb < sp.npb; pb += max(1u, sp.npb - 1u)) {
+      const uint32_t pairs = min(sp.blk, qp - pb * sp.blk), npb_same = (pb + 1 == sp.npb) ? 1u : sp.npb - 1u;
+      if (sp.nrs > 0) atomicAdd(&hist[ms_work_class(ms_row_count(0u, np, rs_rows, rs2_rows), pairs, cls_rows)], npb_same);
+      if (sp.nrs > 2) atomicAdd(&hist[ms_work_class(rs2_rows, pairs, cls_rows)], npb_same * (sp.nrs - 2u));
+      if (sp.nrs > 1) atomicAdd(&hist[ms_work_class(ms_row_count(sp.nrs - 1u, np, rs_rows, rs2_rows), pairs, cls_rows)], npb_same);
+      if (sp.npb == 1) break;
+    }
+  }
+  uint32_t incl = v;
+#pragma unroll
+  for (int off = 1; off < 64; off <<= 1) {
+    const uint32_t t = __shfl_up(incl, off, 64);
+    if (lane >= off) incl += t;
+  }
+  if (lane == 63) wsum[wave] = incl;
+  __syncthreads();
+  uint32_t woff = 0;
+  for (int w = 0; w < wave; ++w) woff += wsum[w];
+  if (i < nlist) { s_start[i] = woff + incl - v; slice_start[i] = woff + incl - v; }
+  if (i == 1023) { s_start[nlist] = woff + incl; slice_start[nlist] = woff + incl; }
+  if (i == 0) {
+    uint32_t run = 0;
+    for (int c = 0; c < 32; ++c) { cur[c] = run; run += hist[c]; }
+  }
+  __syncthreads();
+  const uint32_t total = s_start[nlist];
+  for (uint32_t sl = (uint32_t)i; sl < total; sl += 1024u) {
+    int part = (int)find_partition_dev(s_start, nlist, sl);
+    while (s_start[part + 1] <= sl) ++part;
+    const uint32_t t = sl - s_start[part];
+    const uint32_t off = s_off[part], np = s_np[part], gs = s_gs[part], qp = s_qp[part];
+    const MsSplit sp = ms_split(qp, np, rs_rows, rs2_rows);
+    const uint32_t pb = t / sp.nrs, rs = t - pb * sp.nrs;
+    MsSlice u;
+    u.off = off; u.np = np; u.row_begin = ms_row_begin(rs, rs_rows, rs2_rows); u.row_count = ms_row_count(rs, np, rs_rows, rs2_rows);
+    u.gs = gs + pb * sp.blk; u.qp = min(sp.blk, qp - pb * sp.blk); u.pad0 = u.pad1 = 0u;
+    slices[sl] = u;
+    order[atomicAdd(&cur[ms_work_class(u.row_count, u.qp, cls_rows)], 1u)] = sl;
   }
 }
 
@@ -935,10 +992,15 @@
     const uint32_t rs_rows = (uint32_t)ms_rows_per_slice(), rs2_rows = (uint32_t)ms_rows_per_slice2();
     static const bool no_order = getenv("LANCE_HIP_MS_NOORDER") != nullptr;
     const uint32_t cls_rows = no_order ? 0x40000000u : rs_rows;
+    if (nlist <= MS_SLICES_MAX_NLIST)
+      hipLaunchKernelGGL(ms_slices_kernel, dim3(1), dim3(1024), 0, ctx->stream, pair_starts, ix->part_offsets, nlist, rs_rows, rs2_rows, cls_rows, slice_start,
+                         slice_ctr, slices, order);
+    else {
     hipLaunchKernelGGL(ms_slice_table_kernel, dim3(1), dim3(256), 0, ctx->stream, pair_starts, ix->part_offsets, nlist, rs_rows, rs2_rows, cls_rows, slice_start,
                        slice_ctr, cls_cursor);
     hipLaunchKernelGGL(ms_slice_desc_kernel, dim3((unsigned)cdiv((uint64_t)nlist, 4)), dim3(256), 0, ctx->stream, slice_start, pair_starts, ix->part_offsets,
                        nlist, rs_rows, rs2_rows, cls_rows, slices, cls_cursor, order);
+    }
   }
   ScopedTimer t(ctx, "ivfpq_scan_c1");
   ScopedTimer tm(ctx, "ivfpq_mscan");
diff --git a/lance_amd/csrc/search_pm.hip b/lance_amd/csrc/search_pm.hip
--- a/lance_amd/csrc/search_pm.hip
+++ b/lance_amd/csrc/search_pm.hip
@@ -106,6 +106,39 @@
     dsc.z = i0 + 1 < pe ? (int)(pair_idx[i0 + 1] / (uint32_t)nprobes) : -1;
   }
   desc[item] = dsc;
+}
+
+__global__ __launch_bounds__(256) void pm_items_kernel(const uint32_t *__restrict__ pair_starts, const uint32_t *__restrict__ pair_idx, int nvp, int nlist,
+                                                       int nprobes, uint32_t max_items, uint32_t *__restrict__ item_start, int4 *__restrict__ desc) {
+  __shared__ uint32_t s_start[ITEMS_MAX_NVP + 1];
+  __shared__ uint32_t s_misc[5];
+  item_table_to_lds(pair_starts, nvp, 2, s_start, s_misc, item_start);
+  const uint32_t item = blockIdx.x * 256 + threadIdx.x;
+  if (item >= max_items) return;
+  int4 dsc = make_int4(-1, -1, -1, 0);
+  if (item < s_start[nvp]) {
+    int vp = (int)find_partition_dev(s_start, nvp, item);
+    while (s_start[vp + 1] <= item) ++vp;
+    const uint32_t g = item - s_start[vp];
+    const uint32_t ps = pair_starts[vp], pe = pair_starts[vp + 1];
+    const uint32_t i0 = ps + 2 * g;
+    dsc.x = vp % nlist;
+    dsc.y = (int)(pair_idx[i0] / (uint32_t)nprobes);
+    dsc.z = i0 + 1 < pe ? (int)(pair_idx[i0 + 1] / (uint32_t)nprobes) : -1;
+  }
+  desc[item] = dsc;
+}
+
+static void pm_items_launch(lance_hip_ctx *ctx, const uint32_t *pair_starts, const uint32_t *pair_idx, int nvp, int nlist, int nprobes, uint32_t max_items,
+                            uint32_t *item_start, int4 *desc) {
+  if (nvp <= ITEMS_MAX_NVP && max_items > 0) {
+    hipLaunchKernelGGL(pm_items_kernel, dim3((unsigned)cdiv(max_items, 256)), dim3(256), 0, ctx->stream, pair_starts, pair_idx, nvp, nlist, nprobes, max_items,
+                       item_start, desc);
+    return;
+  }
+  hipLaunchKernelGGL(pm_item_table_kernel, dim3(1), dim3(256), 0, ctx->stream, pair_starts, nvp, item_start);
+  hipLaunchKernelGGL(pm_item_desc_kernel, dim3((unsigned)cdiv(max_items, 256)), dim3(256), 0, ctx->stream, item_start, pair_starts, pair_idx, nvp, nlist, nprobes,
+                     max_items, desc);
 }
 
 template <int SD, int METRIC, int MU, int RPL, int CAP>
@@ -577,12 +610,14 @@
   const bool exact_bound = exact_bound_env && !tiled && !dot;
   {
     ScopedTimer t(ctx, "pm_group");
-    LH_TRY(qscan_nearest_keys(ctx, probes, nq, nprobes, keys, nb0));
-    LH_TRY(stable_group(ctx, keys, (int64_t)nq * nb0, (int64_t)nq * nb0, nlist, 1, pair_starts0, pair_idx0, (int64_t)nq * nb0, nullptr));
+    if (stable_group_small_ok((int64_t)nq * nb0, nlist)) {
+      LH_TRY(stable_group_small(ctx, probes, (int64_t)nq * nb0, (int)nb0, (int64_t)nprobes, nlist, pair_starts0, pair_idx0));
+    } else {
+      LH_TRY(qscan_nearest_keys(ctx, probes, nq, nprobes, keys, nb0));
+      LH_TRY(stable_group(ctx, keys, (int64_t)nq * nb0, (int64_t)nq * nb0, nlist, 1, pair_starts0, pair_idx0, (int64_t)nq * nb0, nullptr));
+    }
     if (exact_bound) {
-      hipLaunchKernelGGL(pm_item_table_kernel, dim3(1), dim3(256), 0, ctx->stream, pair_starts0, nlist, item_start0);
-      hipLaunchKernelGGL(pm_item_desc_kernel, dim3((unsigned)cdiv(max_items0, 256)), dim3(256), 0, ctx->stream, item_start0, pair_starts0, pair_idx0,
-                         nlist, nlist, 1, max_items0, desc0);
+      pm_items_launch(ctx, pair_starts0, pair_idx0, nlist, nlist, 1, max_items0, item_start0, desc0);
     }
   }
   if (exact_bound) {
@@ -605,22 +640,22 @@
     if (mb_rc == LH_NOT_TAKEN && dot) return LH_NOT_TAKEN;
     if (mb_rc == LH_NOT_TAKEN) LH_TRY(qbound_launch(ctx, ix, qs, nq, keff, pair_starts0, pair_idx0, item_start0, desc0, (uint32_t)(nq / 4 + nlist + 2), tglobal, allow));
   }
+  const bool ms_expected = mscan_supported(ix, nq, nprobes);
   {
     ScopedTimer t(ctx, "pm_group");
-    LH_TRY(qscan_group(ctx, probes, nq, nprobes, nlist, tglobal, keys, tbound, pair_starts, pair_idx, item_start4, desc4, max_items4, 4, dot ? 1 : 0));
-    hipLaunchKernelGGL(pm_item_table_kernel, dim3(1), dim3(256), 0, ctx->stream, pair_starts, 2 * nlist, item_start);
-    hipLaunchKernelGGL(pm_item_desc_kernel, dim3((unsigned)cdiv(max_items2, 256)), dim3(256), 0, ctx->stream, item_start, pair_starts, pair_idx,
-                       2 * nlist, nlist, (int)nprobes, max_items2, desc);
+    LH_TRY(qscan_group(ctx, probes, nq, nprobes, nlist, tglobal, keys, tbound, pair_starts, pair_idx, ms_expected ? nullptr : item_start4, desc4, max_items4, 4, dot ? 1 : 0));
+    pm_items_launch(ctx, pair_starts, pair_idx, 2 * nlist, nlist, (int)nprobes, max_items2, item_start, desc);
   }
   uint32_t *qslack = nullptr;
   float *seg_val = nullptr, *seg_scale = nullptr;
   int ms_rc = LH_NOT_TAKEN;
-  if (mscan_supported(ix, nq, nprobes))
+  if (ms_expected)
     ms_rc = mscan_launch(ctx, ix, qs, nq, nprobes, probes, pair_starts, pair_idx, tbound, seg_cnt, seg_pos, qovf, allow, &qslack, &seg_val, &seg_scale);
   if (ms_rc < 0) return ms_rc;
   if (ms_rc == LH_NOT_TAKEN && dot) return LH_NOT_TAKEN;
   if (ms_rc == LH_NOT_TAKEN) {
     qslack = nullptr; seg_val = nullptr; seg_scale = nullptr;
+    if (ms_expected) LH_TRY(qscan_item_tables(ctx, pair_starts, nlist, 4, item_start4, desc4, max_items4));
     LH_TRY(qscan_launch(ctx, ix, qs, nq, nprobes, pair_idx, item_start4, desc4, max_items4, tbound, seg_cnt, seg_pos, qovf, allow, probes));
   }
   static const bool q_stats = getenv("LANCE_HIP_Q_STATS") != nullptr;
@@ -689,9 +724,7 @@
     hipLaunchKernelGGL(pm_keys_kernel, dim3((unsigned)cdiv(npairs, 256)), dim3(256), 0, ctx->stream, probes, (int64_t)npairs, (int)nprobes,
                        nlist, keys);
     LH_TRY(stable_group(ctx, keys, (int64_t)npairs, (int64_t)npairs, 2 * nlist, 1, pair_starts, pair_idx, (int64_t)npairs, nullptr));
-    hipLaunchKernelGGL(pm_item_table_kernel, dim3(1), dim3(256), 0, ctx->stream, pair_starts, 2 * nlist, item_start);
-    hipLaunchKernelGGL(pm_item_desc_kernel, dim3((unsigned)cdiv(max_items, 256)), dim3(256), 0, ctx->stream, item_start, pair_starts, pair_idx,
-                       2 * nlist, nlist, (int)nprobes, max_items, desc);
+    pm_items_launch(ctx, pair_starts, pair_idx, 2 * nlist, nlist, (int)nprobes, max_items, item_start, desc);
   }
   PmArgs a;
   a.q = qs; a.probes = probes; a.pair_starts = pair_starts; a.pair_idx = pair_idx; a.item_start = item_start;
diff --git a/lance_amd/csrc/search_q.hip b/lance_amd/csrc/search_q.hip
--- a/lance_amd/csrc/search_q.hip
+++ b/lance_amd/csrc/search_q.hip
@@ -68,6 +68,27 @@
     int vp = (int)find_partition_dev(item_start, nvp, item);
     while (item_start[vp + 1] <= item) ++vp;
     const uint32_t g = item - item_start[vp];
+    const uint32_t ps = pair_starts[vp], pe = pair_starts[vp + 1];
+    const uint32_t i0 = ps + (uint32_t)G * g;
+    dsc.x = vp;
+    dsc.y = (int)i0;
+    dsc.z = (int)min((uint32_t)G, pe - i0);
+  }
+  desc[item] = dsc;
+}
+
+__global__ __launch_bounds__(256) void q_items_kernel(const uint32_t *__restrict__ pair_starts, int nvp, int G, uint32_t max_items,
+                                                      uint32_t *__restrict__ item_start, int4 *__restrict__ desc) {
+  __shared__ uint32_t s_start[ITEMS_MAX_NVP + 1];
+  __shared__ uint32_t s_misc[5];
+  item_table_to_lds(pair_starts, nvp, G, s_start, s_misc, item_start);
+  const uint32_t item = blockIdx.x * 256 + threadIdx.x;
+  if (item >= max_items) return;
+  int4 dsc = make_int4(-1, 0, 0, 0);
+  if (item < s_start[nvp]) {
+    int vp = (int)find_partition_dev(s_start, nvp, item);
+    while (s_start[vp + 1] <= item) ++vp;
+    const uint32_t g = item - s_start[vp];
     const uint32_t ps = pair_starts[vp], pe = pair_starts[vp + 1];
     const uint32_t i0 = ps + (uint32_t)G * g;
     dsc.x = vp;
@@ -1023,13 +1044,15 @@
   hipLaunchKernelGGL(q_tclass_keys_kernel, dim3((unsigned)cdiv(npairs, 256)), dim3(256), 0, ctx->stream, probes, (int64_t)npairs, (int)nprobes,
                      nlist, tglobal, keys, tbound, dot);
   LH_TRY(stable_group(ctx, keys, (int64_t)npairs, (int64_t)npairs, 2 * nlist, 1, pair_starts, pair_idx, (int64_t)npairs, nullptr));
-  hipLaunchKernelGGL(q_item_table_kernel, dim3(1), dim3(256), 0, ctx->stream, pair_starts, nlist, G, item_start4);
-  hipLaunchKernelGGL(q_item_desc_kernel, dim3((unsigned)cdiv(max_items4, 256)), dim3(256), 0, ctx->stream, item_start4, pair_starts, nlist, G,
-                     max_items4, desc4);
+  if (item_start4) return qscan_item_tables(ctx, pair_starts, nlist, G, item_start4, desc4, max_items4);
   return LANCE_HIP_OK;
 }
 
 int qscan_item_tables(lance_hip_ctx *ctx, const uint32_t *pair_starts, int nlist, int G, uint32_t *item_start, int4 *desc, uint32_t max_items) {
+  if (nlist <= ITEMS_MAX_NVP && max_items > 0) {
+    hipLaunchKernelGGL(q_items_kernel, dim3((unsigned)cdiv(max_items, 256)), dim3(256), 0, ctx->stream, pair_starts, nlist, G, max_items, item_start, desc);
+    return LANCE_HIP_OK;
+  }
   hipLaunchKernelGGL(q_item_table_kernel, dim3(1), dim3(256), 0, ctx->stream, pair_starts, nlist, G, item_start);
   hipLaunchKernelGGL(q_item_desc_kernel, dim3((unsigned)cdiv(max_items, 256)), dim3(256), 0, ctx->stream, item_start, pair_starts, nlist, G, max_items, desc);
   return LANCE_HIP_OK;
@@ -1148,8 +1171,7 @@
 }
 
 int qscan_items(lance_hip_ctx *ctx, const uint32_t *pair_starts, int nvp, int G, uint32_t *item_start, int4 *desc, uint32_t max_items) {
-  hipLaunchKernelGGL(q_item_table_kernel, dim3(1), dim3(256), 0, ctx->stream, pair_starts, nvp, G, item_start);
-  hipLaunchKernelGGL(q_item_desc_kernel, dim3((unsigned)cdiv(max_items, 256)), dim3(256), 0, ctx->stream, item_start, pair_starts, nvp, G, max_items, desc);
+  LH_TRY(qscan_item_tables(ctx, pair_starts, nvp, G, item_start, desc, max_items));
   LH_CHECK_HIP(hipGetLastError());
   return LANCE_HIP_OK;
 }
@@ -1157,9 +1179,7 @@
 int qbound_launch(lance_hip_ctx *ctx, const lance_hip_index *ix, const float *qs, uint32_t nq, uint32_t keff, const uint32_t *pair_starts0,
                   const uint32_t *pair_idx0, uint32_t *item_start, int4 *desc, uint32_t max_items, uint32_t *tglobal, const uint32_t *allow) {
   const int d = (int)ix->d, m = (int)ix->m, sd = d / m, nlist = (int)ix->nlist;
-  hipLaunchKernelGGL(q_item_table_kernel, dim3(1), dim3(256), 0, ctx->stream, pair_starts0, nlist, Q_G, item_start);
-  hipLaunchKernelGGL(q_item_desc_kernel, dim3((unsigned)cdiv(max_items, 256)), dim3(256), 0, ctx->stream, item_start, pair_starts0, nlist, Q_G,
-                     max_items, desc);
+  LH_TRY(qscan_item_tables(ctx, pair_starts0, nlist, Q_G, item_start, desc, max_items));
   f4 *rq = reinterpret_cast<f4 *>(ctx->scratch_t<float>("qbound.rq", (size_t)max_items * d * 4));
   if (!rq) return LANCE_HIP_ENOMEM;
   hipLaunchKernelGGL(q_residual_kernel, dim3((unsigned)cdiv(max_items, 4)), dim3(256), 0, ctx->stream, qs, pair_idx0, item_start, desc, ix->centroids, d,
```

Result: faster. 25.58 million queries/s, median of 6 (+1.4%).
